# mozilla/mozjpeg

Measured on NVIDIA H100. Metric: megapixels/sec encode (4K RGB q75 4:2:0), higher is better.
Workload: dtype u8 in / int32 DCT / fp32 trellis costs / u8 out

## Files before the change

mozjpeg_b200/csrc/kernels.cu:

```cuda
#include "kernels.cuh"
#include <cuda_fp16.h>
#include <cuda.h>
#include <cstdio>
#include <cstdlib>
#include <type_traits>

namespace b200 {

unsigned long long g_kernel_launches = 0;
#define LAUNCHED() (++g_kernel_launches)

__constant__ uint8_t c_zz[64] = {
   0,  1,  8, 16,  9,  2,  3, 10, 17, 24, 32, 25, 18, 11,  4,  5,
  12, 19, 26, 33, 40, 48, 41, 34, 27, 20, 13,  6,  7, 14, 21, 28,
  35, 42, 49, 56, 57, 50, 43, 36, 29, 22, 15, 23, 30, 37, 44, 51,
  58, 59, 52, 45, 38, 31, 39, 46, 53, 60, 61, 54, 47, 55, 62, 63};
__constant__ uint8_t c_izz[64] = {
   0,  1,  5,  6, 14, 15, 27, 28,  2,  4,  7, 13, 16, 26, 29, 42,
   3,  8, 12, 17, 25, 30, 41, 43,  9, 11, 18, 24, 31, 40, 44, 53,
  10, 19, 23, 32, 39, 45, 52, 54, 20, 22, 33, 38, 46, 51, 55, 60,
  21, 34, 37, 47, 50, 56, 59, 61, 35, 36, 48, 49, 57, 58, 62, 63};
__constant__ unsigned long long c_izz_col[8] = {0x2315140a09030200ull, 0x242216130b080401ull, 0x30252117120c0705ull, 0x312f262018110d06ull, 0x39322e271f19100eull, 0x3a38332d281e1a0full, 0x3e3b37342c291d1bull, 0x3f3d3c36352b2a1cull};
#ifndef FWD_KZ_PACKED
#define FWD_KZ_PACKED 1
#endif
#define ZZ_LIST \
  X(0,0) X(1,1) X(2,8) X(3,16) X(4,9) X(5,2) X(6,3) X(7,10) X(8,17) X(9,24) X(10,32) X(11,25) X(12,18) X(13,11) X(14,4) X(15,5) \
  X(16,12) X(17,19) X(18,26) X(19,33) X(20,40) X(21,48) X(22,41) X(23,34) X(24,27) X(25,20) X(26,13) X(27,6) X(28,7) X(29,14) X(30,21) X(31,28) \
  X(32,35) X(33,42) X(34,49) X(35,56) X(36,57) X(37,50) X(38,43) X(39,36) X(40,29) X(41,22) X(42,15) X(43,23) X(44,30) X(45,37) X(46,44) X(47,51) \
  X(48,58) X(49,59) X(50,52) X(51,45) X(52,38) X(53,31) X(54,39) X(55,46) X(56,53) X(57,60) X(58,61) X(59,54) X(60,47) X(61,55) X(62,62) X(63,63)

#define NAT_LIST Y(1,1) Y(2,5) Y(3,6) Y(4,14) Y(5,15) Y(6,27) Y(7,28) Y(8,2) Y(9,4) Y(10,7) Y(11,13) Y(12,16) Y(13,26) Y(14,29) Y(15,42) Y(16,3) Y(17,8) Y(18,12) Y(19,17) Y(20,25) Y(21,30) Y(22,41) Y(23,43) Y(24,9) Y(25,11) Y(26,18) Y(27,24) Y(28,31) Y(29,40) Y(30,44) Y(31,53) Y(32,10) Y(33,19) Y(34,23) Y(35,32) Y(36,39) Y(37,45) Y(38,52) Y(39,54) Y(40,20) Y(41,22) Y(42,33) Y(43,38) Y(44,46) Y(45,51) Y(46,55) Y(47,60) Y(48,21) Y(49,34) Y(50,37) Y(51,47) Y(52,50) Y(53,56) Y(54,59) Y(55,61) Y(56,35) Y(57,36) Y(58,48) Y(59,49) Y(60,57) Y(61,58) Y(62,62) Y(63,63)

__device__ __forceinline__ int nbits_of(int v) { return 32 - __clz(v); }

template <int SB>
__device__ __forceinline__ int convert_sample(const uint8_t *__restrict__ px, int cs_mode, int comp, int first, int swap)
{
  constexpr int MAXJ = SB == 1 ? 255 : 4095, CENTRE = (MAXJ + 1) / 2;
  auto smp = [&](int k) -> int { return SB == 1 ? (int)px[k] : (int)(reinterpret_cast<const uint16_t *>(px)[k] & 0xFFF); };
  if (cs_mode == 2 || comp == 3) {
    const int k = first + (swap ? 2 - comp : comp);
    return SB == 1 || cs_mode == 2 ? smp(k) : (int)reinterpret_cast<const uint16_t *>(px)[k];
  }
  const int inv = cs_mode == 3 ? MAXJ : 0;
  const int r = smp(first + (swap ? 2 : 0)) ^ inv, g = smp(first + 1) ^ inv, b = smp(first + (swap ? 0 : 2)) ^ inv;
  if (comp == 0) return (19595 * r + 38470 * g + 7471 * b + 32768) >> 16;
  if (comp == 1) return (-11059 * r - 21709 * g + 32768 * b + (CENTRE << 16) + 32767) >> 16;
  return (32768 * r - 27439 * g - 5329 * b + (CENTRE << 16) + 32767) >> 16;
}

#define DESCALE(x, n) (((x) + (1 << ((n) - 1))) >> (n))
template <int PASS, int P1 = 2>
__device__ __forceinline__ void fdct_1d(int &d0, int &d1, int &d2, int &d3, int &d4, int &d5, int &d6, int &d7)
{
  int t0 = d0 + d7, t7 = d0 - d7, t1 = d1 + d6, t6 = d1 - d6;
  int t2 = d2 + d5, t5 = d2 - d5, t3 = d3 + d4, t4 = d3 - d4;
  int t10 = t0 + t3, t13 = t0 - t3, t11 = t1 + t2, t12 = t1 - t2;
  constexpr int SH = PASS == 0 ? 13 - P1 : 13 + P1;
  if (PASS == 0) { d0 = (t10 + t11) << P1; d4 = (t10 - t11) << P1; }
  else { d0 = DESCALE(t10 + t11, P1); d4 = DESCALE(t10 - t11, P1); }
  int z1 = (t12 + t13) * 4433;
  d2 = DESCALE(z1 + t13 * 6270, SH);
  d6 = DESCALE(z1 + t12 * (-15137), SH);
  z1 = t4 + t7; int z2 = t5 + t6, z3 = t4 + t6, z4 = t5 + t7;
  int z5 = (z3 + z4) * 9633;
  t4 *= 2446; t5 *= 16819; t6 *= 25172; t7 *= 12299;
  z1 *= -7373; z2 *= -20995; z3 *= -16069; z4 *= -3196;
  z3 += z5; z4 += z5;
  d7 = DESCALE(t4 + z1 + z3, SH);
  d5 = DESCALE(t5 + z2 + z4, SH);
  d3 = DESCALE(t6 + z2 + z3, SH);
  d1 = DESCALE(t7 + z1 + z4, SH);
}

__device__ __forceinline__ float catmull_rom(int v1, int v2, int v3, int v4, float t, int size)
{
  const int tan1 = (v3 - v1) * size, tan2 = (v4 - v2) * size;
  const float t2 = t * t, t3 = t2 * t;
  const float f1 = 2.f * t3 - 3.f * t2 + 1.f;
  const float f2 = -2.f * t3 + 3.f * t2;
  const float f3 = t3 - 2.f * t2 + t;
  const float f4 = t3 - t2;
  return (float)v2 * f1 + (float)tan1 * f3 + (float)v3 * f2 + (float)tan2 * f4;
}
template <class Acc>
__device__ __forceinline__ void deringing_block(Acc A, int q0, int sum, int cnt)
{
  const int maxsample = 127, size = 64;
  int m = min(min(31, 2 * q0), (maxsample * size - sum) / cnt);
  int maxover = maxsample + m;
  int n = 0;
  do {
    if (A.get(c_zz[n]) < maxsample) { n++; continue; }
    int start = n;
    while (++n < size && A.get(c_zz[n]) >= maxsample) {}
    int end = n;
    int f1 = A.get(c_zz[start >= 1 ? start - 1 : 0]);
    int f2 = A.get(c_zz[start >= 2 ? start - 2 : 0]);
    int l1 = A.get(c_zz[end < size - 1 ? end : size - 1]);
    int l2 = A.get(c_zz[end < size - 2 ? end + 1 : size - 1]);
    int fslope = max(f1 - f2, maxsample - f1);
    int lslope = max(l1 - l2, maxsample - l1);
    if (start == 0) fslope = lslope;
    if (end == size) lslope = fslope;
    int length = end - start;
    float step = 1.f / (float)(length + 1);
    float position = step;
    for (int i = start; i < end; i++, position += step) {
      int tmp = (int)ceilf(catmull_rom(maxsample - fslope, maxsample, maxsample, maxsample - lslope, position, length));
      A.set(c_zz[i], min(tmp, maxover));
    }
    n++;
  } while (n < size);
}
struct LocalAcc { int *d; __device__ int get(int n) const { return d[n]; } __device__ void set(int n, int v) const { d[n] = v; } };
struct PlaneAcc {
  int16_t *p; int pitch;
  __device__ int get(int n) const { return p[(n >> 3) * pitch + (n & 7)]; }
  __device__ void set(int n, int v) const { p[(n >> 3) * pitch + (n & 7)] = (int16_t)v; }
};

__device__ __forceinline__ unsigned quant_one(int x, QuantConst k, int dering)
{
  unsigned a = (unsigned)abs(x) + k.bias;
  int q = (int)(((unsigned long long)a * k.mul) >> k.shift);
  if (dering) q = min(q, 1023);
  return (unsigned)(x < 0 ? -q : q);
}

__device__ __forceinline__ void fdct_ifast_1d(int &d0, int &d1, int &d2, int &d3, int &d4, int &d5, int &d6, int &d7)
{
  int tmp0 = d0 + d7, tmp7 = d0 - d7, tmp1 = d1 + d6, tmp6 = d1 - d6;
  int tmp2 = d2 + d5, tmp5 = d2 - d5, tmp3 = d3 + d4, tmp4 = d3 - d4;
  int tmp10 = tmp0 + tmp3, tmp13 = tmp0 - tmp3, tmp11 = tmp1 + tmp2, tmp12 = tmp1 - tmp2;
  d0 = tmp10 + tmp11; d4 = tmp10 - tmp11;
  int z1 = ((tmp12 + tmp13) * 181) >> 8;
  d2 = tmp13 + z1; d6 = tmp13 - z1;
  tmp10 = tmp4 + tmp5; tmp11 = tmp5 + tmp6; tmp12 = tmp6 + tmp7;
  int z5 = ((tmp10 - tmp12) * 98) >> 8;
  int z2 = ((tmp10 * 139) >> 8) + z5;
  int z4 = ((tmp12 * 334) >> 8) + z5;
  int z3 = (tmp11 * 181) >> 8;
  int z11 = tmp7 + z3, z13 = tmp7 - z3;
  d5 = z13 + z2; d3 = z13 - z2; d1 = z11 + z4; d7 = z11 - z4;
}
__constant__ short c_aanscales[64] = {
  16384, 22725, 21407, 19266, 16384, 12873,  8867,  4520,
  22725, 31521, 29692, 26722, 22725, 17855, 12299,  6270,
  21407, 29692, 27969, 25172, 21407, 16819, 11585,  5906,
  19266, 26722, 25172, 22654, 19266, 15137, 10426,  5315,
  16384, 22725, 21407, 19266, 16384, 12873,  8867,  4520,
  12873, 17855, 16819, 15137, 12873, 10114,  6967,  3552,
   8867, 12299, 11585, 10426,  8867,  6967,  4799,  2446,
   4520,  6270,  5906,  5315,  4520,  3552,  2446,  1247};

__device__ __forceinline__ void fdct_float_1d(float &d0, float &d1, float &d2, float &d3, float &d4, float &d5, float &d6, float &d7)
{
  float tmp0 = d0 + d7, tmp7 = d0 - d7, tmp1 = d1 + d6, tmp6 = d1 - d6;
  float tmp2 = d2 + d5, tmp5 = d2 - d5, tmp3 = d3 + d4, tmp4 = d3 - d4;
  float tmp10 = tmp0 + tmp3, tmp13 = tmp0 - tmp3, tmp11 = tmp1 + tmp2, tmp12 = tmp1 - tmp2;
  d0 = tmp10 + tmp11; d4 = tmp10 - tmp11;
  float z1 = (tmp12 + tmp13) * 0.707106781f;
  d2 = tmp13 + z1; d6 = tmp13 - z1;
  tmp10 = tmp4 + tmp5; tmp11 = tmp5 + tmp6; tmp12 = tmp6 + tmp7;
  float z5 = (tmp10 - tmp12) * 0.382683433f;
  float z2 = 0.541196100f * tmp10 + z5;
  float z4 = 1.306562965f * tmp12 + z5;
  float z3 = tmp11 * 0.707106781f;
  float z11 = tmp7 + z3, z13 = tmp7 - z3;
  d5 = z13 + z2; d3 = z13 - z2; d1 = z11 + z4; d7 = z11 - z4;
}
__device__ __forceinline__ void deringing_block_float(float *data, int q0, float sum, int cnt)
{
  const float maxsample = 127.0f; const int size = 64;
  const int a = min(31, 2 * q0); const float bq = (maxsample * size - sum) / (float)cnt;
  const float maxovershoot = maxsample + ((float)a < bq ? (float)a : bq);
  int n = 0;
  do {
    if (data[c_zz[n]] < maxsample) { n++; continue; }
    int start = n;
    while (++n < size && data[c_zz[n]] >= maxsample) {}
    int end = n;
    float f1 = data[c_zz[start >= 1 ? start - 1 : 0]], f2 = data[c_zz[start >= 2 ? start - 2 : 0]];
    float l1 = data[c_zz[end < size - 1 ? end : size - 1]], l2 = data[c_zz[end < size - 2 ? end + 1 : size - 1]];
    float fslope = fmaxf(f1 - f2, maxsample - f1), lslope = fmaxf(l1 - l2, maxsample - l1);
    if (start == 0) fslope = lslope;
    if (end == size) lslope = fslope;
    int length = end - start;
    float step = 1.f / (float)(length + 1), position = step;
    for (int i = start; i < end; i++, position += step) {
      float tmp = catmull_rom((int)(maxsample - fslope), 127, 127, (int)(maxsample - lslope), position, length);
      data[c_zz[i]] = tmp < maxovershoot ? tmp : maxovershoot;
    }
    n++;
  } while (n < size);
}
__constant__ double c_aan[8] = {1.0, 1.387039845, 1.306562965, 1.175875602, 1.0, 0.785694958, 0.541196100, 0.275899379};

__device__ __forceinline__ unsigned qc_d(const QuantTables *__restrict__ qt, int t, int i) { return qt->q[t][i].d; }
template <int PREC, int DCTM>
__global__ void __launch_bounds__(128) k_forward(Geom g, const uint8_t *__restrict__ src,
                                                 const QuantTables *__restrict__ qt, int dering,
                                                 DcRec *__restrict__ rec, RecLayout rl)
{
  constexpr int CENTRE = 1 << (PREC - 1);
  constexpr int SB = PREC == 8 ? 1 : 2;
  constexpr int P1 = PREC == 8 ? 2 : 1;
  const int ci = blockIdx.z % g.nc, img = blockIdx.z / g.nc;
  const CompGeom &c = g.c[ci];
  int bx = blockIdx.x * blockDim.x + threadIdx.x;
  int by = blockIdx.y;
  if (bx >= c.wib || by >= c.hib) return;
  auto set = [&] { return qset_of(qt, g, img); };
  const uint8_t *base = src + (size_t)img * g.image_stride;
  int ws[64];
  const int comp = g.cs_mode == 1 ? 0 : ci;
  auto component = [&](const uint8_t *px) -> int { return convert_sample<SB>(px, g.cs_mode, comp, g.px_first, g.px_swap); };
#pragma unroll
  for (int y = 0; y < 8; y++) {
    int yo = by * 8 + y;
    int yy = min(yo, c.rows_avail - 1);
    int grp = yy / c.v, sub = yy - grp * c.v;
    int iy0 = grp * g.vmax + sub * c.vx;
#pragma unroll
    for (int x = 0; x < 8; x++) {
      int xo = bx * 8 + x;
      if (g.raw_in) {
        const uint8_t *q = g.plane[ci] + (size_t)img * g.plane_stride[ci] + (size_t)yo * g.plane_pitch[ci] + (size_t)xo * SB;
        ws[8 * y + x] = (SB == 1 ? (int)*q : (int)*reinterpret_cast<const uint16_t *>(q)) - CENTRE;
        continue;
      }
      int sum = 0;
      for (int dv = 0; dv < c.vx; dv++) {
        int iy = min(iy0 + dv, g.H - 1);
        const uint8_t *row = base + (size_t)iy * g.row_pitch;
        for (int du = 0; du < c.hx; du++) {
          int ix = min(xo * c.hx + du, g.W - 1);
          sum += component(row + (size_t)ix * g.in_comps * SB);
        }
      }
      int val;
      if (c.hx == 1 && c.vx == 1) val = sum;
      else if (c.hx == 2 && c.vx == 1) val = (sum + (xo & 1)) >> 1;
      else if (c.hx == 2 && c.vx == 2) val = (sum + 1 + (xo & 1)) >> 2;
      else { int np = c.hx * c.vx; val = (sum + np / 2) / np; }
      ws[8 * y + x] = val - CENTRE;
    }
  }
  int qv[64];
  if (DCTM == 2) {
    float wf[64];
    int sum = 0, cnt = 0;
#pragma unroll
    for (int i = 0; i < 64; i++) { wf[i] = (float)ws[i]; sum += ws[i]; cnt += (ws[i] >= 127); }
    if (dering && cnt != 0 && cnt != 64) deringing_block_float(wf, (int)set()->q[c.qt][0].d >> 3, (float)sum, cnt);
#pragma unroll
    for (int r = 0; r < 8; r++) fdct_float_1d(wf[8 * r], wf[8 * r + 1], wf[8 * r + 2], wf[8 * r + 3], wf[8 * r + 4], wf[8 * r + 5], wf[8 * r + 6], wf[8 * r + 7]);
#pragma unroll
    for (int col = 0; col < 8; col++) fdct_float_1d(wf[col], wf[8 + col], wf[16 + col], wf[24 + col], wf[32 + col], wf[40 + col], wf[48 + col], wf[56 + col]);
    const float *fd = set()->fdiv[c.qt];
#pragma unroll
    for (int i = 0; i < 64; i++) {
      float v = wf[i];
      v = (float)((double)v / c_aan[i & 7]);
      v = (float)((double)v / c_aan[i >> 3]);
      ws[i] = (v >= 0.0f) ? (int)((double)v + 0.5) : (int)((double)v - 0.5);
      int q = (int)(int16_t)(__float2int_rz(wf[i] * fd[i] + 16384.5f) - 16384);
      if (dering) q = max(-1023, min(1023, q));
      qv[i] = q;
    }
  } else {
    if (dering) {
      int sum = 0, cnt = 0;
#pragma unroll
      for (int i = 0; i < 64; i++) { sum += ws[i]; cnt += (ws[i] >= 127); }
      if (cnt != 0 && cnt != 64) {
        int tmp[64];
#pragma unroll
        for (int i = 0; i < 64; i++) tmp[i] = ws[i];
        deringing_block(LocalAcc{tmp}, (int)set()->q[c.qt][0].d >> 3, sum, cnt);
#pragma unroll
        for (int i = 0; i < 64; i++) ws[i] = tmp[i];
      }
    }
    if (DCTM == 1) {
#pragma unroll
      for (int r = 0; r < 8; r++) fdct_ifast_1d(ws[8 * r], ws[8 * r + 1], ws[8 * r + 2], ws[8 * r + 3], ws[8 * r + 4], ws[8 * r + 5], ws[8 * r + 6], ws[8 * r + 7]);
#pragma unroll
      for (int col = 0; col < 8; col++) fdct_ifast_1d(ws[col], ws[8 + col], ws[16 + col], ws[24 + col], ws[32 + col], ws[40 + col], ws[48 + col], ws[56 + col]);
      const IfastConst *ic = set()->ifast[c.qt];
#pragma unroll
      for (int i = 0; i < 64; i++) {
        const int x = ws[i], sc = c_aanscales[i];
        const int a = abs(x);
        int q;
        if (PREC == 8) {
          const IfastConst k = ic[i];
          q = (int)(int16_t)(int)(((unsigned long long)(unsigned)(a + (int)k.corr) * k.recip) >> (k.shift + 32));
        } else {
          const int d = (int)(((long long)((int)qc_d(set(), c.qt, i) >> 3) * sc + (1 << 10)) >> 11);
          q = (int)(int16_t)((a + (d >> 1)) / d);
        }
        if (x < 0) q = (int)(int16_t)(-q);
        if (dering) q = max(-1023, min(1023, q));
        qv[i] = q;
        ws[i] = (int)((x >= 0) ? ((long long)x * 32768 + sc) / (2 * sc) : ((long long)x * 32768 - sc) / (2 * sc));
      }
    } else {
#pragma unroll
      for (int r = 0; r < 8; r++)
        fdct_1d<0, P1>(ws[8 * r], ws[8 * r + 1], ws[8 * r + 2], ws[8 * r + 3], ws[8 * r + 4], ws[8 * r + 5], ws[8 * r + 6], ws[8 * r + 7]);
#pragma unroll
      for (int col = 0; col < 8; col++)
        fdct_1d<1, P1>(ws[col], ws[8 + col], ws[16 + col], ws[24 + col], ws[32 + col], ws[40 + col], ws[48 + col], ws[56 + col]);
    }
  }
  const QuantConst *qc = set()->q[c.qt];
  if (rec) {
    float norm = 0.0f; unsigned long long mask = 0;
#pragma unroll
    for (int i = 1; i < 64; i++) {
      norm += (float)(ws[i] * ws[i]);
      bool nz;
      if (DCTM == 0) nz = quant_one(ws[i], qc[i], dering) != 0u;
      else { const int dq = (int)qc[i].d; nz = abs(ws[i]) >= dq - dq / 2; }
      if (nz) mask |= 1ull << c_izz[i];
    }
    DcRec rr; rr.lambda_dc = norm; rr.raw_dc = (int16_t)ws[0]; rr.nz = (uint8_t)__popcll(mask); rr.pad = 0; rr.nzmask = mask;
    rec[(size_t)img * rl.per_image + rl.comp_off[ci] + (size_t)by * c.wib + bx] = rr;
  }
  size_t blk = ((size_t)img * c.hpad + by) * c.wpad + bx;
  uint4 *dq = reinterpret_cast<uint4 *>(c.coef + blk * 64);
  uint4 *dr = reinterpret_cast<uint4 *>(c.raw + blk * 64);
  unsigned pq[32], pr[32];
#define X(k, n) { unsigned qq = (DCTM == 0 ? quant_one(ws[n], qc[n], dering) : (unsigned)qv[n]) & 0xFFFFu, rr = (unsigned)ws[n] & 0xFFFFu; \
                  if ((k) & 1) { pq[(k) >> 1] |= qq << 16; pr[(k) >> 1] |= rr << 16; } else { pq[(k) >> 1] = qq; pr[(k) >> 1] = rr; } }
  ZZ_LIST
#undef X
#pragma unroll
  for (int v = 0; v < 8; v++) {
    dq[v] = make_uint4(pq[4 * v], pq[4 * v + 1], pq[4 * v + 2], pq[4 * v + 3]);
    dr[v] = make_uint4(pr[4 * v], pr[4 * v + 1], pr[4 * v + 2], pr[4 * v + 3]);
  }
}

template <int PREC> struct WorkT { typedef int16_t type; };
template <> struct WorkT<12> { typedef int type; };
template <> struct WorkT<32> { typedef float type; };
struct Px8 { unsigned w[12]; };
template <int IC, int SB>
__device__ __forceinline__ Px8 load_px8(const uint8_t *__restrict__ base, size_t row_pitch, int iy, int x, int W, bool fast, bool px4 = false, int first = 0)
{
  Px8 r;
  const uint8_t *row = base + (size_t)iy * row_pitch;
  constexpr int NBYTES = 8 * IC * SB;
#pragma unroll
  for (int i = 0; i < 12; i++) r.w[i] = 0;
  if (fast && IC == 3 && px4) {
    unsigned q[16];
    if (SB == 1) {
      const uint4 *p = reinterpret_cast<const uint4 *>(row + (size_t)x * 4);
      const uint4 a = __ldg(p), b = __ldg(p + 1);
      q[0] = a.x; q[1] = a.y; q[2] = a.z; q[3] = a.w; q[4] = b.x; q[5] = b.y; q[6] = b.z; q[7] = b.w;
      if (first) {
#pragma unroll
        for (int i = 0; i < 8; i++) q[i] >>= 8;
      }
#pragma unroll
      for (int g4 = 0; g4 < 2; g4++) {
        const unsigned p0 = q[4 * g4], p1 = q[4 * g4 + 1], p2 = q[4 * g4 + 2], p3 = q[4 * g4 + 3];
        r.w[3 * g4] = __byte_perm(p0, p1, 0x4210);
        r.w[3 * g4 + 1] = __byte_perm(p1, p2, 0x5421);
        r.w[3 * g4 + 2] = __byte_perm(p2, p3, 0x6542);
      }
    } else {
      const uint4 *p = reinterpret_cast<const uint4 *>(row + (size_t)x * 8);
#pragma unroll
      for (int i = 0; i < 4; i++) { const uint4 a = __ldg(p + i); q[4 * i] = a.x; q[4 * i + 1] = a.y; q[4 * i + 2] = a.z; q[4 * i + 3] = a.w; }
#pragma unroll
      for (int k = 0; k < 8; k++) {
        const unsigned lo = q[2 * k], hi = q[2 * k + 1];
        const unsigned c0 = first ? (lo >> 16) : (lo & 0xFFFFu), c1 = first ? (hi & 0xFFFFu) : (lo >> 16), c2 = first ? (hi >> 16) : (hi & 0xFFFFu);
        const unsigned cc[3] = {c0, c1, c2};
#pragma unroll
        for (int c = 0; c < 3; c++) { const int h = 3 * k + c; r.w[h >> 1] |= cc[c] << (16 * (h & 1)); }
      }
    }
    return r;
  }
  if (fast) {
    if (SB == 1) {
      const uint2 *p = reinterpret_cast<const uint2 *>(row + (size_t)x * IC);
#pragma unroll
      for (int i = 0; i < NBYTES / 8; i++) { uint2 a = __ldg(p + i); r.w[2 * i] = a.x; r.w[2 * i + 1] = a.y; }
    } else {
      const uint4 *p = reinterpret_cast<const uint4 *>(row + (size_t)x * IC * 2);
#pragma unroll
      for (int i = 0; i < NBYTES / 16; i++) { uint4 a = __ldg(p + i); r.w[4 * i] = a.x; r.w[4 * i + 1] = a.y; r.w[4 * i + 2] = a.z; r.w[4 * i + 3] = a.w; }
    }
  } else {
    const int pxb = (IC == 3 && px4 ? 4 : IC) * SB, off = (IC == 3 && px4 ? first : 0) * SB;
#pragma unroll
    for (int b = 0; b < NBYTES; b++) {
      int px = b / (IC * SB), rem = b - px * (IC * SB);
      int ix = min(x + px, W - 1);
      r.w[b >> 2] |= (unsigned)row[(size_t)ix * pxb + off + rem] << (8 * (b & 3));
    }
  }
  return r;
}
template <int IC, int SB>
__device__ __forceinline__ int px_sample(const Px8 &r, int px, int ch)
{
  if (SB == 1) { int b = px * IC + ch; return (int)__byte_perm(r.w[b >> 2], 0u, 0x4440 | (b & 3)); }
  int h = px * IC + ch; return (int)((r.w[h >> 1] >> (16 * (h & 1))) & 0xFFFu);
}

__device__ __forceinline__ int quant_fast(int x, uint2 k, int L, int dering)
{
  unsigned a14 = (unsigned)abs(x) * 16384u + k.y;
  int q = (int)(__umulhi(a14, k.x) >> L);
  if (dering) q = min(q, 1023);
  return x < 0 ? -q : q;
}


#ifndef FWD_MASK_SQ
#define FWD_MASK_SQ 1
#endif
#ifndef FWD_MIN_CTAS
#define FWD_MIN_CTAS 6
#endif
template <int HMAX, int VMAX, int NC, bool QFAST, int PREC, int DCTM>
__global__ void __launch_bounds__(128, FWD_MIN_CTAS) k_forward_tile(Geom g, const uint8_t *__restrict__ src,
                                                      const QuantTables *__restrict__ qt, int dering,
                                                      DcRec *__restrict__ rec, RecLayout rl, int write_raw, FwdStats fs,
                                                      const __grid_constant__ CUtensorMap tmap, const int use_tma)
{
  constexpr int TW = 128, TR = 8 * VMAX;
  constexpr int YBW = TW / 8, YB = YBW * VMAX;
  constexpr int CW = TW / HMAX, CBW = CW / 8;
  constexpr int NB = YB + (NC == 3 ? 2 * CBW : 0);
  constexpr int YP = TW + 8, CP = CW + 8;
  constexpr int IC = NC == 3 ? 3 : 1;
  constexpr int SB = PREC == 8 ? 1 : 2;
  constexpr int P1 = PREC == 8 ? 2 : 1;
  constexpr int CENTRE = 1 << (PREC - 1);
  typedef typename WorkT<DCTM == 2 ? 32 : PREC>::type wtype;
  __shared__ __align__(16) int16_t sY[TR * YP];
  __shared__ __align__(16) int16_t sC[NC == 3 ? 2 * 8 * CP : 8];
  __shared__ __align__(16) wtype sW[NB * 72];
  __shared__ __align__(128) unsigned char sIO[NB * 256];
  __shared__ __align__(8) unsigned long long tma_bar;
  __shared__ uint2 sQC[NC][64];
  __shared__ uint2 sMask[NB];
  __shared__ int sQL[NC];
  __shared__ unsigned sHist[NC][HIST_BINS];

  const int tid = threadIdx.x;
  const int tx = blockIdx.x, ty = blockIdx.y, img = blockIdx.z;
  const int x0 = tx * TW, y0 = ty * TR;
  const uint8_t *base = src + (size_t)img * g.image_stride;
  qt = qset_of(qt, g, img);
  if (fs.hist) for (int i = tid; i < NC * HIST_BINS; i += 128) (&sHist[0][0])[i] = 0;

  for (int i = tid; i < NC * 64; i += 128) { int ci = i >> 6, n = i & 63; const QuantConst &k = qt->q[g.c[ci].qt][n]; sQC[ci][n] = make_uint2(k.mul2, k.bias << 14); }
  if (tid < NC) sQL[tid] = qt->L[g.c[tid].qt];

  constexpr int TMA_BOXW = IC == 3 ? 192 : 128, TMA_NBOX = IC == 3 ? 2 : 1;
  static_assert(TMA_NBOX * TMA_BOXW * TR <= NB * 256, "the pixel tile fits the staging buffer it borrows");
  const bool tma_tile = PREC == 8 && use_tma && x0 + TW <= g.W && y0 + TR <= g.H;
  if (tma_tile) {
    const unsigned bar = (unsigned)__cvta_generic_to_shared(&tma_bar);
    if (tid == 0) {
      asm volatile("mbarrier.init.shared::cta.b64 [%0], 1;" :: "r"(bar) : "memory");
      asm volatile("fence.mbarrier_init.release.cluster;" ::: "memory");
      asm volatile("mbarrier.arrive.expect_tx.shared::cta.b64 _, [%0], %1;" :: "r"(bar), "r"((unsigned)(TMA_NBOX * TMA_BOXW * TR)) : "memory");
#pragma unroll
      for (int bx = 0; bx < TMA_NBOX; bx++)
        asm volatile("cp.async.bulk.tensor.3d.shared::cluster.global.mbarrier::complete_tx::bytes [%0], [%1, {%2, %3, %4}], [%5];"
                     :: "r"((unsigned)__cvta_generic_to_shared(sIO + bx * TMA_BOXW * TR)), "l"(reinterpret_cast<unsigned long long>(&tmap)),
                        "r"(x0 * IC + bx * TMA_BOXW), "r"(y0), "r"(g.image_stride ? img : 0), "r"(bar) : "memory");
    }
    __syncthreads();
    {
      unsigned done = 0;
      while (!done)
        asm volatile("{ .reg .pred p; mbarrier.try_wait.parity.shared::cta.b64 p, [%1], 0; selp.u32 %0, 1, 0, p; }" : "=r"(done) : "r"(bar) : "memory");
    }
  }

  {
    const int rg = tid >> 4, seg = tid & 15;
    const int xs = x0 + seg * 8;
    auto tma_px8 = [&](int trow) {
      Px8 r;
#pragma unroll
      for (int i = 0; i < 12; i++) r.w[i] = 0;
      if (IC == 3) {
        const uint2 *q = reinterpret_cast<const uint2 *>(sIO + (seg >> 3) * (TMA_BOXW * TR) + trow * TMA_BOXW + (seg & 7) * 24);
#pragma unroll
        for (int i = 0; i < 3; i++) { const uint2 a = q[i]; r.w[2 * i] = a.x; r.w[2 * i + 1] = a.y; }
      } else {
        const uint2 a = *reinterpret_cast<const uint2 *>(sIO + trow * TMA_BOXW + seg * 8);
        r.w[0] = a.x; r.w[1] = a.y;
      }
      return r;
    };
    if (g.raw_in) {
      auto sample = [&](int cc, int row, int x) -> int {
        const uint8_t *q = g.plane[cc] + (size_t)img * g.plane_stride[cc] + (size_t)row * g.plane_pitch[cc] + (size_t)x * SB;
        return SB == 1 ? (int)*q : (int)*reinterpret_cast<const uint16_t *>(q);
      };
#pragma unroll
      for (int rr = 0; rr < VMAX; rr++) {
        const int row = y0 + rg * VMAX + rr;
        const CompGeom &c0 = g.c[0];
        int16_t yv[8];
#pragma unroll
        for (int px = 0; px < 8; px++) {
          const int x = xs + px;
          yv[px] = (row < c0.hib * 8 && x < c0.wib * 8) ? (int16_t)(sample(0, row, x) - CENTRE) : (int16_t)0;
        }
        *reinterpret_cast<uint4 *>(&sY[(rg * VMAX + rr) * YP + seg * 8]) = *reinterpret_cast<const uint4 *>(yv);
      }
      if (NC == 3) {
        const int row = ty * 8 + rg;
#pragma unroll
        for (int cc = 1; cc <= 2; cc++) {
          const CompGeom &c1 = g.c[cc];
          int16_t cv[8 / HMAX];
#pragma unroll
          for (int i = 0; i < 8 / HMAX; i++) {
            const int x = x0 / HMAX + seg * (8 / HMAX) + i;
            cv[i] = (row < c1.hib * 8 && x < c1.wib * 8) ? (int16_t)(sample(cc, row, x) - CENTRE) : (int16_t)0;
          }
          int16_t *dst = &sC[(cc - 1) * 8 * CP + rg * CP + seg * (8 / HMAX)];
          if (HMAX == 1) *reinterpret_cast<uint4 *>(dst) = *reinterpret_cast<const uint4 *>(cv);
          else *reinterpret_cast<uint2 *>(dst) = *reinterpret_cast<const uint2 *>(cv);
        }
      }
    } else {
    const bool grey_from_rgb = NC == 1 && g.cs_mode == 1;
    const bool px4 = g.in_comps == 4 && (NC == 3 || grey_from_rgb);
    const int pfirst = g.px_first; const bool pswap = g.px_swap != 0;
    const size_t AL = px4 ? 15 : (SB == 1 ? 7 : 15);
    const bool fast = (xs + 8 <= g.W) && ((g.row_pitch & AL) == 0) && ((((size_t)base) & AL) == 0) && !grey_from_rgb;
    if (NC == 1 && grey_from_rgb) {
#pragma unroll
      for (int rr = 0; rr < VMAX; rr++) {
        const int iy = min(y0 + rg * VMAX + rr, g.H - 1);
        const bool f3 = (xs + 8 <= g.W) && ((g.row_pitch & AL) == 0) && ((((size_t)base) & AL) == 0);
        Px8 p = load_px8<3, SB>(base, g.row_pitch, iy, xs, g.W, f3, px4, pfirst);
        int16_t yv[8];
#pragma unroll
        for (int px = 0; px < 8; px++) {
          const int s0 = px_sample<3, SB>(p, px, 0), s2 = px_sample<3, SB>(p, px, 2);
          yv[px] = (int16_t)(((19595 * (pswap ? s2 : s0) + 38470 * px_sample<3, SB>(p, px, 1) + 7471 * (pswap ? s0 : s2) + 32768) >> 16) - CENTRE);
        }
        *reinterpret_cast<uint4 *>(&sY[(rg * VMAX + rr) * YP + seg * 8]) = *reinterpret_cast<const uint4 *>(yv);
      }
    } else {
      auto convert = [&](auto ext_tag) {
      constexpr bool EXT = decltype(ext_tag)::value;
      int sb[8 / HMAX], sr[8 / HMAX];
#pragma unroll
      for (int i = 0; i < 8 / HMAX; i++) { sb[i] = 0; sr[i] = 0; }
      const int last_real = NC == 3 ? g.c[1].rows_avail - 1 - ty * 8 : 8;
      const int er = min(rg, last_real);
#pragma unroll
      for (int rr = 0; rr < VMAX; rr++) {
        const int iy = min(y0 + rg * VMAX + rr, g.H - 1);
        Px8 p = (!EXT && tma_tile) ? tma_px8(rg * VMAX + rr) : load_px8<IC, SB>(base, g.row_pitch, iy, xs, g.W, fast, EXT && px4, EXT ? pfirst : 0);
        int16_t yv[8];
#pragma unroll
        for (int px = 0; px < 8; px++) {
          if (NC == 1) yv[px] = (int16_t)(px_sample<1, SB>(p, px, 0) - CENTRE);
          else {
            const int S0 = px_sample<3, SB>(p, px, 0), G = px_sample<3, SB>(p, px, 1), S2 = px_sample<3, SB>(p, px, 2);
            const int R = (EXT && pswap) ? S2 : S0, B = (EXT && pswap) ? S0 : S2;
            yv[px] = (int16_t)(((19595 * R + 38470 * G + 7471 * B + 32768) >> 16) - CENTRE);
          }
        }
        *reinterpret_cast<uint4 *>(&sY[(rg * VMAX + rr) * YP + seg * 8]) = *reinterpret_cast<const uint4 *>(yv);
        if (NC == 3) {
          if (er != rg) p = (!EXT && tma_tile) ? tma_px8(er * VMAX + rr) : load_px8<IC, SB>(base, g.row_pitch, min(y0 + er * VMAX + rr, g.H - 1), xs, g.W, fast, EXT && px4, EXT ? pfirst : 0);
#pragma unroll
          for (int px = 0; px < 8; px++) {
            const int S0 = px_sample<3, SB>(p, px, 0), G = px_sample<3, SB>(p, px, 1), S2 = px_sample<3, SB>(p, px, 2);
            const int R = (EXT && pswap) ? S2 : S0, B = (EXT && pswap) ? S0 : S2;
            sb[px / HMAX] += (-11059 * R - 21709 * G + 32768 * B + (CENTRE << 16) + 32767) >> 16;
            sr[px / HMAX] += (32768 * R - 27439 * G - 5329 * B + (CENTRE << 16) + 32767) >> 16;
          }
        }
      }
      if (NC == 3) {
        int16_t cbv[8 / HMAX], crv[8 / HMAX];
#pragma unroll
        for (int i = 0; i < 8 / HMAX; i++) {
          const int xo = x0 / HMAX + seg * (8 / HMAX) + i;
          int b = sb[i], r = sr[i];
          if (HMAX == 2 && VMAX == 1) { b = (b + (xo & 1)) >> 1; r = (r + (xo & 1)) >> 1; }
          else if (HMAX == 2 && VMAX == 2) { b = (b + 1 + (xo & 1)) >> 2; r = (r + 1 + (xo & 1)) >> 2; }
          else if (HMAX * VMAX > 1) { b = (b + HMAX * VMAX / 2) / (HMAX * VMAX); r = (r + HMAX * VMAX / 2) / (HMAX * VMAX); }
          cbv[i] = (int16_t)(b - CENTRE); crv[i] = (int16_t)(r - CENTRE);
        }
        int16_t *cb = &sC[rg * CP + seg * (8 / HMAX)], *cr = &sC[8 * CP + rg * CP + seg * (8 / HMAX)];
        if (HMAX == 1) { *reinterpret_cast<uint4 *>(cb) = *reinterpret_cast<const uint4 *>(cbv); *reinterpret_cast<uint4 *>(cr) = *reinterpret_cast<const uint4 *>(crv); }
        else { *reinterpret_cast<uint2 *>(cb) = *reinterpret_cast<const uint2 *>(cbv); *reinterpret_cast<uint2 *>(cr) = *reinterpret_cast<const uint2 *>(crv); }
      }
      };
      if (px4 || pswap) convert(std::true_type{}); else convert(std::false_type{});
    }
    }
  }
  __syncthreads();

  const int j = tid & 7;
#pragma unroll 1
  for (int b = tid >> 3; b < NB; b += 16) {
    int16_t *plane; int pitch, bx, byl;
    if (b < YB) { plane = sY; pitch = YP; byl = b / YBW; bx = b - byl * YBW; }
    else { int cb = b - YB; int which = cb / CBW; plane = sC + which * 8 * CP; pitch = CP; byl = 0; bx = cb - which * CBW; }
    int16_t *rowp = plane + (byl * 8 + j) * pitch + bx * 8;
    const uint4 rv = *reinterpret_cast<const uint4 *>(rowp);
    int d0 = (int)(int16_t)(rv.x & 0xFFFF), d1 = (int)rv.x >> 16, d2 = (int)(int16_t)(rv.y & 0xFFFF), d3 = (int)rv.y >> 16;
    int d4 = (int)(int16_t)(rv.z & 0xFFFF), d5 = (int)rv.z >> 16, d6 = (int)(int16_t)(rv.w & 0xFFFF), d7 = (int)rv.w >> 16;
    if (DCTM == 2) {
      float f0 = (float)d0, f1 = (float)d1, f2 = (float)d2, f3 = (float)d3, f4 = (float)d4, f5 = (float)d5, f6 = (float)d6, f7 = (float)d7;
      float *w = reinterpret_cast<float *>(sW) + b * 72 + j * 8;
      if (dering) {
        int sum = d0 + d1 + d2 + d3 + d4 + d5 + d6 + d7;
        int cnt = (d0 >= 127) + (d1 >= 127) + (d2 >= 127) + (d3 >= 127) + (d4 >= 127) + (d5 >= 127) + (d6 >= 127) + (d7 >= 127);
        sum += __shfl_xor_sync(0xffffffffu, sum, 1); cnt += __shfl_xor_sync(0xffffffffu, cnt, 1);
        sum += __shfl_xor_sync(0xffffffffu, sum, 2); cnt += __shfl_xor_sync(0xffffffffu, cnt, 2);
        sum += __shfl_xor_sync(0xffffffffu, sum, 4); cnt += __shfl_xor_sync(0xffffffffu, cnt, 4);
        if (cnt != 0 && cnt != 64) {
          w[0] = f0; w[1] = f1; w[2] = f2; w[3] = f3; w[4] = f4; w[5] = f5; w[6] = f6; w[7] = f7;
          __syncwarp(0xFFu << (threadIdx.x & 24));
          if (j == 0) {
            const int ci = b < YB ? 0 : (1 + (b - YB) / CBW);
            deringing_block_float(reinterpret_cast<float *>(sW) + b * 72, (int)qt->q[g.c[ci].qt][0].d >> 3, (float)sum, cnt);
          }
          __syncwarp(0xFFu << (threadIdx.x & 24));
          f0 = w[0]; f1 = w[1]; f2 = w[2]; f3 = w[3]; f4 = w[4]; f5 = w[5]; f6 = w[6]; f7 = w[7];
        }
      }
      fdct_float_1d(f0, f1, f2, f3, f4, f5, f6, f7);
      w[0] = f0; w[1] = f1; w[2] = f2; w[3] = f3; w[4] = f4; w[5] = f5; w[6] = f6; w[7] = f7;
      continue;
    }
    if (dering) {
      int sum = d0 + d1 + d2 + d3 + d4 + d5 + d6 + d7;
      int cnt = (d0 >= 127) + (d1 >= 127) + (d2 >= 127) + (d3 >= 127) + (d4 >= 127) + (d5 >= 127) + (d6 >= 127) + (d7 >= 127);
      sum += __shfl_xor_sync(0xffffffffu, sum, 1); cnt += __shfl_xor_sync(0xffffffffu, cnt, 1);
      sum += __shfl_xor_sync(0xffffffffu, sum, 2); cnt += __shfl_xor_sync(0xffffffffu, cnt, 2);
      sum += __shfl_xor_sync(0xffffffffu, sum, 4); cnt += __shfl_xor_sync(0xffffffffu, cnt, 4);
      if (cnt != 0 && cnt != 64) {
        if (j == 0) {
          const int ci = b < YB ? 0 : (1 + (b - YB) / CBW);
          deringing_block(PlaneAcc{plane + (byl * 8) * pitch + bx * 8, pitch}, (int)qt->q[g.c[ci].qt][0].d >> 3, sum, cnt);
        }
        __syncwarp(0xFFu << (threadIdx.x & 24));
        d0 = rowp[0]; d1 = rowp[1]; d2 = rowp[2]; d3 = rowp[3]; d4 = rowp[4]; d5 = rowp[5]; d6 = rowp[6]; d7 = rowp[7];
      }
    }
    if (DCTM == 1) fdct_ifast_1d(d0, d1, d2, d3, d4, d5, d6, d7);
    else fdct_1d<0, P1>(d0, d1, d2, d3, d4, d5, d6, d7);
    if (DCTM == 2) {
    } else if (PREC == 8) {
      uint4 wv;
      wv.x = ((unsigned)d0 & 0xFFFFu) | ((unsigned)d1 << 16); wv.y = ((unsigned)d2 & 0xFFFFu) | ((unsigned)d3 << 16);
      wv.z = ((unsigned)d4 & 0xFFFFu) | ((unsigned)d5 << 16); wv.w = ((unsigned)d6 & 0xFFFFu) | ((unsigned)d7 << 16);
      *reinterpret_cast<uint4 *>(reinterpret_cast<int16_t *>(sW) + b * 72 + j * 8) = wv;
    } else {
      int *w = reinterpret_cast<int *>(sW) + b * 72 + j * 8;
      w[0] = d0; w[1] = d1; w[2] = d2; w[3] = d3; w[4] = d4; w[5] = d5; w[6] = d6; w[7] = d7;
    }
  }
  __syncthreads();

  int16_t *sQ = reinterpret_cast<int16_t *>(sIO);
  int16_t *sR = sQ + NB * 64;
  static_assert(NB % 16 == 0, "whole warps walk the block list in step");
  const int jc = (j + 2 * ((tid >> 3) & 3)) & 7;
  int kz[8];
#pragma unroll
  for (int r = 0; r < 8; r++) {
#if FWD_KZ_PACKED
    kz[r] = (int)((c_izz_col[jc] >> (8 * r)) & 63);
#else
    kz[r] = c_izz[8 * r + jc];
#endif
  }
#pragma unroll 1
  for (int b = tid >> 3; b < NB; b += 16) {
    const wtype *w = sW + b * 72 + jc;
    const int ci = b < YB ? 0 : (1 + (b - YB) / CBW);
    int dd[8], qf[8];
    if (DCTM == 2) {
      float f0 = w[0], f1 = w[8], f2 = w[16], f3 = w[24], f4 = w[32], f5 = w[40], f6 = w[48], f7 = w[56];
      fdct_float_1d(f0, f1, f2, f3, f4, f5, f6, f7);
      const float ff[8] = {f0, f1, f2, f3, f4, f5, f6, f7};
      const float *fd = qt->fdiv[g.c[ci].qt];
#pragma unroll
      for (int r = 0; r < 8; r++) {
        dd[r] = 0;
        if (write_raw) {
          float v = ff[r];
          v = (float)((double)v / c_aan[jc]);
          v = (float)((double)v / c_aan[r]);
          dd[r] = (v >= 0.0f) ? (int)((double)v + 0.5) : (int)((double)v - 0.5);
        }
        const float temp = ff[r] * fd[8 * r + jc];
        int q = (int)(int16_t)(__float2int_rz(temp + 16384.5f) - 16384);
        if (dering) q = max(-1023, min(1023, q));
        qf[r] = q;
      }
    } else if (DCTM == 1) {
      int d0 = w[0], d1 = w[8], d2 = w[16], d3 = w[24], d4 = w[32], d5 = w[40], d6 = w[48], d7 = w[56];
      fdct_ifast_1d(d0, d1, d2, d3, d4, d5, d6, d7);
      const int ws8[8] = {d0, d1, d2, d3, d4, d5, d6, d7};
      const IfastConst *ic = qt->ifast[g.c[ci].qt];
#pragma unroll
      for (int r = 0; r < 8; r++) {
        const int nat = 8 * r + jc;
        dd[r] = 0;
        if (write_raw) { const int x = ws8[r], sc = c_aanscales[nat]; dd[r] = (x >= 0) ? (x * 32768 + sc) / (2 * sc) : (x * 32768 - sc) / (2 * sc); }
        const IfastConst k = ic[nat];
        const int a = abs(ws8[r]);
        int q = (int)(int16_t)(int)(((unsigned long long)(unsigned)(a + (int)k.corr) * k.recip) >> (k.shift + 32));
        if (ws8[r] < 0) q = (int)(int16_t)(-q);
        if (dering) q = max(-1023, min(1023, q));
        qf[r] = q;
      }
    } else {
      int d0 = w[0], d1 = w[8], d2 = w[16], d3 = w[24], d4 = w[32], d5 = w[40], d6 = w[48], d7 = w[56];
      fdct_1d<1, P1>(d0, d1, d2, d3, d4, d5, d6, d7);
      dd[0] = d0; dd[1] = d1; dd[2] = d2; dd[3] = d3; dd[4] = d4; dd[5] = d5; dd[6] = d6; dd[7] = d7;
    }
    const int L = sQL[NC == 1 ? 0 : ci];
    unsigned mlo = 0, mhi = 0;
#pragma unroll
    for (int r = 0; r < 8; r++) {
      const int nat = 8 * r + jc;
      const int k = kz[r];
      int qv;
      if (DCTM != 0) qv = qf[r];
      else if (QFAST) qv = quant_fast(dd[r], sQC[NC == 1 ? 0 : ci][nat], L, dering);
      else qv = (int)(int16_t)quant_one(dd[r], qt->q[g.c[ci].qt][nat], dering);
      sQ[b * 64 + k] = (int16_t)qv;
      sR[b * 64 + k] = (int16_t)dd[r];
      if (!(FWD_MASK_SQ && DCTM == 0)) {
        bool nzv = qv != 0;
        if (DCTM != 0 && rec) { const int dq = (int)qt->q[g.c[ci].qt][nat].d; nzv = abs(dd[r]) >= dq - dq / 2; }
        if (nzv && nat != 0) { if (k < 32) mlo |= 1u << k; else mhi |= 1u << (k - 32); }
      }
    }
    if (PREC == 8 && rec) {
      if (DCTM == 2) __syncwarp();
      int16_t *blk16 = reinterpret_cast<int16_t *>(sW + b * 72);
      int16_t *ww = blk16 + jc;
#pragma unroll
      for (int r = 0; r < 8; r++) ww[8 * r] = (int16_t)dd[r];
      if (FWD_MASK_SQ && DCTM == 0) {
        __syncwarp();
        const uint4 zq = *reinterpret_cast<const uint4 *>(sQ + b * 64 + 8 * j);
        const unsigned zw[4] = {zq.x, zq.y, zq.z, zq.w};
        unsigned m8 = 0;
#pragma unroll
        for (int i = 0; i < 4; i++) {
          const unsigned nz = (((zw[i] & 0x7FFF7FFFu) + 0x7FFF7FFFu) | zw[i]) & 0x80008000u;
          const unsigned t2 = nz >> 15;
          m8 |= ((t2 | (t2 >> 15)) & 3u) << (2 * i);
        }
        if (j == 0) m8 &= ~1u;
        reinterpret_cast<uint8_t *>(&sMask[b])[j] = (uint8_t)m8;
      } else {
      mlo |= __shfl_xor_sync(0xffffffffu, mlo, 1); mhi |= __shfl_xor_sync(0xffffffffu, mhi, 1);
      mlo |= __shfl_xor_sync(0xffffffffu, mlo, 2); mhi |= __shfl_xor_sync(0xffffffffu, mhi, 2);
      mlo |= __shfl_xor_sync(0xffffffffu, mlo, 4); mhi |= __shfl_xor_sync(0xffffffffu, mhi, 4);
      if (j == 0) sMask[b] = make_uint2(mlo, mhi);
      }
    }
  }
  asm volatile("fence.proxy.async.shared::cta;" ::: "memory");
  __syncthreads();

  if (PREC == 8 && rec) {
    for (int b = tid; b < NB; b += 128) {
      int ci, row, col;
      if (b < YB) { ci = 0; int byl = b / YBW; row = ty * VMAX + byl; col = tx * YBW + (b - byl * YBW); }
      else { int cb = b - YB; int which = cb / CBW; ci = 1 + which; row = ty; col = tx * CBW + (cb - which * CBW); }
      const CompGeom &c = g.c[ci];
      if (row >= c.hib || col >= c.wib) continue;
      const int4 *rows = reinterpret_cast<const int4 *>(reinterpret_cast<const int16_t *>(sW + b * 72));
      float norm = 0.0f; int raw_dc = 0;
      const float bias = -8421376.0f;
#pragma unroll
      for (int r = 0; r < 8; r++) {
        const int4 rv = rows[r];
        const unsigned pw[4] = {(unsigned)rv.x, (unsigned)rv.y, (unsigned)rv.z, (unsigned)rv.w};
#pragma unroll
        for (int cp = 0; cp < 4; cp++) {
          const unsigned u = pw[cp] ^ 0x80008000u;
          float2 f = make_float2(__fadd_rn(__uint_as_float(__byte_perm(u, 0x4B000000u, 0x7610)), bias),
                                 __fadd_rn(__uint_as_float(__byte_perm(u, 0x4B000000u, 0x7632)), bias));
          f.x = __fmul_rn(f.x, f.x); f.y = __fmul_rn(f.y, f.y);
          if (r == 0 && cp == 0) raw_dc = (int)(int16_t)(pw[0] & 0xFFFFu); else norm += f.x;
          norm += f.y;
        }
      }
      const uint2 mk = sMask[b];
      DcRec rr; rr.lambda_dc = norm; rr.raw_dc = (int16_t)raw_dc; rr.nz = (uint8_t)(__popc(mk.x) + __popc(mk.y)); rr.pad = 0;
      rr.nzmask = ((unsigned long long)mk.y << 32) | mk.x;
      const size_t ridx = (size_t)img * rl.per_image + rl.comp_off[ci] + (size_t)row * c.wib + col;
      rec[ridx] = rr;
      if (fs.hist) {
        const int16_t *q = sQ + b * 64;
        fs.dcq[ridx] = q[0];
        unsigned long long m;
        if (FWD_MASK_SQ && DCTM == 0) m = rr.nzmask;
        else {
          m = 0;
#pragma unroll
          for (int v = 0; v < 8; v++) {
            const uint4 zq = reinterpret_cast<const uint4 *>(q)[v];
            const unsigned zw[4] = {zq.x, zq.y, zq.z, zq.w};
#pragma unroll
            for (int i = 0; i < 4; i++) {
              const unsigned nz = (((zw[i] & 0x7FFF7FFFu) + 0x7FFF7FFFu) | zw[i]) & 0x80008000u;
              const unsigned t2 = nz >> 15;
              m |= (unsigned long long)((t2 | (t2 >> 15)) & 3u) << (8 * v + 2 * i);
            }
          }
          m &= ~1ull;
        }
        unsigned *h = sHist[NC == 1 ? 0 : ci];
        if (!(m >> 63)) atomicAdd(&h[0], 1u);
        int prev = 0; bool bad = false;
        while (m) {
          const int k = __ffsll((long long)m) - 1;
          m &= m - 1;
          const int run = k - prev - 1; prev = k;
          const int nb = nbits_of(abs((int)q[k]));
          bad |= nb > g.max_coef_bits;
          if (run >> 4) atomicAdd(&h[0xF0], (unsigned)(run >> 4));
          atomicAdd(&h[((run & 15) << 4) + nb], 1u);
        }
        if (bad) atomicOr(&fs.status[img], 2u);
      }
    }
  }

  if (PREC == 8 && fs.hist) {
    __syncthreads();
    for (int i = tid; i < NC * HIST_BINS; i += 128) {
      const unsigned v = (&sHist[0][0])[i];
      const int ci = i / HIST_BINS, sym = i - ci * HIST_BINS;
      if (v) atomicAdd(&fs.hist[(((size_t)img * g.nc + ci) * HIST_SLOTS + 4 + g.c[ci].ac_tbl) * HIST_BINS + sym], v);
    }
  }

  {
    constexpr int NRUN = VMAX + (NC == 3 ? 2 : 0);
    if (tid < NRUN) {
      int ci, row, col0, b0, maxblk;
      if (tid < VMAX) { ci = 0; row = ty * VMAX + tid; col0 = tx * YBW; b0 = tid * YBW; maxblk = YBW; }
      else { const int which = tid - VMAX; ci = 1 + which; row = ty; col0 = tx * CBW; b0 = YB + which * CBW; maxblk = CBW; }
      const CompGeom &c = g.c[ci];
      const int cnt = row < c.hib ? max(0, min(maxblk, c.wib - col0)) : 0;
      if (cnt > 0) {
        const size_t blk = ((size_t)img * c.hpad + row) * c.wpad + col0;
        const unsigned bytes = (unsigned)cnt * 128u;
        if (!fs.hist)
          asm volatile("cp.async.bulk.global.shared::cta.bulk_group [%0], [%1], %2;"
                       :: "l"(c.coef + blk * 64), "r"((unsigned)__cvta_generic_to_shared(sQ + b0 * 64)), "r"(bytes) : "memory");
        if (write_raw)
          asm volatile("cp.async.bulk.global.shared::cta.bulk_group [%0], [%1], %2;"
                       :: "l"(c.raw + blk * 64), "r"((unsigned)__cvta_generic_to_shared(sR + b0 * 64)), "r"(bytes) : "memory");
        asm volatile("cp.async.bulk.commit_group;" ::: "memory");
        asm volatile("cp.async.bulk.wait_group.read 0;" ::: "memory");
      }
    }
  }
}

typedef CUresult (*EncodeTiledFn)(CUtensorMap *, CUtensorMapDataType, cuuint32_t, void *, const cuuint64_t *, const cuuint64_t *, const cuuint32_t *,
                                  const cuuint32_t *, CUtensorMapInterleave, CUtensorMapSwizzle, CUtensorMapL2promotion, CUtensorMapFloatOOBfill);
static EncodeTiledFn tensor_map_encoder()
{
  static EncodeTiledFn fn = [] {
    void *p = nullptr; cudaDriverEntryPointQueryResult q;
    if (cudaGetDriverEntryPoint("cuTensorMapEncodeTiled", &p, cudaEnableDefault, &q) != cudaSuccess || q != cudaDriverEntryPointSuccess) p = nullptr;
    return reinterpret_cast<EncodeTiledFn>(p);
  }();
  return fn;
}
static int make_pixel_tensor_map(const Geom &g, const uint8_t *src, int n, int ic, int tile_rows, CUtensorMap *tm)
{
  static const bool off = getenv("B200JPEG_NO_TMA") != nullptr;
  memset(tm, 0, sizeof *tm);
  EncodeTiledFn enc = tensor_map_encoder();
  if (off || !enc || g.raw_in || !src || g.in_comps != ic || g.px_swap || g.px_first || g.max_coef_bits != 10) return 0;
  if (g.image_stride == 0) n = 1;
  if (((size_t)src & 15) || (g.row_pitch & 15) || (n > 1 && (g.image_stride & 15))) return 0;
  const cuuint64_t dims[3] = {(cuuint64_t)g.W * ic, (cuuint64_t)g.H, (cuuint64_t)n};
  const cuuint64_t strides[2] = {(cuuint64_t)g.row_pitch, (cuuint64_t)(n > 1 ? g.image_stride : ((g.row_pitch * (size_t)g.H + 15) & ~(size_t)15))};
  const cuuint32_t box[3] = {(cuuint32_t)(ic == 3 ? 192 : 128), (cuuint32_t)tile_rows, 1};
  const cuuint32_t estr[3] = {1, 1, 1};
  return enc(tm, CU_TENSOR_MAP_DATA_TYPE_UINT8, 3, const_cast<uint8_t *>(src), dims, strides, box, estr, CU_TENSOR_MAP_INTERLEAVE_NONE,
             CU_TENSOR_MAP_SWIZZLE_NONE, CU_TENSOR_MAP_L2_PROMOTION_L2_128B, CU_TENSOR_MAP_FLOAT_OOB_FILL_NONE) == CUDA_SUCCESS;
}

template <bool QFAST, int PREC, int DCTM>
static void launch_forward_tile(const Geom &g, const uint8_t *src, const QuantTables *qt, int dering, DcRec *rec, const RecLayout &rl, const FwdStats &fs, int n, cudaStream_t s, bool gray, int write_raw)
{
  dim3 grid((g.W + 127) / 128, g.mcu_rows, n);
  CUtensorMap tm;
  const int use_tma = PREC == 8 ? make_pixel_tensor_map(g, src, n, gray ? 1 : 3, 8 * (gray ? 1 : g.vmax), &tm) : (memset(&tm, 0, sizeof tm), 0);
  if (gray) k_forward_tile<1, 1, 1, QFAST, PREC, DCTM><<<grid, 128, 0, s>>>(g, src, qt, dering, rec, rl, write_raw, fs, tm, use_tma);
  else if (g.hmax == 1 && g.vmax == 1) k_forward_tile<1, 1, 3, QFAST, PREC, DCTM><<<grid, 128, 0, s>>>(g, src, qt, dering, rec, rl, write_raw, fs, tm, use_tma);
  else if (g.hmax == 2 && g.vmax == 1) k_forward_tile<2, 1, 3, QFAST, PREC, DCTM><<<grid, 128, 0, s>>>(g, src, qt, dering, rec, rl, write_raw, fs, tm, use_tma);
  else if (g.hmax == 1 && g.vmax == 2) k_forward_tile<1, 2, 3, QFAST, PREC, DCTM><<<grid, 128, 0, s>>>(g, src, qt, dering, rec, rl, write_raw, fs, tm, use_tma);
  else k_forward_tile<2, 2, 3, QFAST, PREC, DCTM><<<grid, 128, 0, s>>>(g, src, qt, dering, rec, rl, write_raw, fs, tm, use_tma);
}
template <int SB>
__global__ void __launch_bounds__(128) k_prep_planes(Geom g, const uint8_t *__restrict__ src, int sf, PlanesOut out)
{
  const int ci = blockIdx.z % g.nc, img = blockIdx.z / g.nc;
  const CompGeom &c = g.c[ci];
  const int xo = blockIdx.x * blockDim.x + threadIdx.x, yo = blockIdx.y;
  if (xo >= c.wib * 8 || yo >= c.hib * 8) return;
  const uint8_t *base = src + (size_t)img * g.image_stride;
  const int comp = g.cs_mode == 1 ? 0 : ci;
  auto at = [&](int y, int x) -> int {
    y = max(0, min(y, g.H - 1)); x = max(0, min(x, g.W - 1));
    return convert_sample<SB>(base + (size_t)y * g.row_pitch + (size_t)x * g.in_comps * SB, g.cs_mode, comp, g.px_first, g.px_swap);
  };
  int val;
  if (c.hx == 1 && c.vx == 1) {
    const int member = at(yo, xo);
    int neigh = -member;
    for (int dy = -1; dy <= 1; dy++) for (int dx = -1; dx <= 1; dx++) neigh += at(yo + dy, xo + dx);
    val = (member * (65536 - sf * 512) + neigh * (sf * 64) + 32768) >> 16;
  } else if (c.hx == 2 && c.vx == 2) {
    const int y = 2 * yo, x = 2 * xo;
    const int member = at(y, x) + at(y, x + 1) + at(y + 1, x) + at(y + 1, x + 1);
    int edge = at(y - 1, x) + at(y - 1, x + 1) + at(y + 2, x) + at(y + 2, x + 1) + at(y, x - 1) + at(y, x + 2) + at(y + 1, x - 1) + at(y + 1, x + 2);
    const int corner = at(y - 1, x - 1) + at(y - 1, x + 2) + at(y + 2, x - 1) + at(y + 2, x + 2);
    val = (member * (16384 - sf * 80) + (2 * edge + corner) * (sf * 16) + 32768) >> 16;
  } else {
    int sum = 0;
    for (int dv = 0; dv < c.vx; dv++) for (int du = 0; du < c.hx; du++) sum += at(yo * c.vx + dv, xo * c.hx + du);
    if (c.hx == 2 && c.vx == 1) val = (sum + (xo & 1)) >> 1;
    else { const int np = c.hx * c.vx; val = (sum + np / 2) / np; }
  }
  uint8_t *dst = out.p[ci] + (size_t)img * out.stride[ci] + (size_t)yo * out.pitch[ci] + (size_t)xo * SB;
  if (SB == 1) *dst = (uint8_t)val; else *reinterpret_cast<uint16_t *>(dst) = (uint16_t)val;
}
void launch_prep_planes(const Geom &g, const uint8_t *src, int smoothing_factor, const PlanesOut &out, int n, cudaStream_t s)
{
  int mw = 0, mh = 0;
  for (int ci = 0; ci < g.nc; ci++) { mw = max(mw, g.c[ci].wib * 8); mh = max(mh, g.c[ci].hib * 8); }
  dim3 grid((mw + 127) / 128, mh, n * g.nc);
  if (g.max_coef_bits == 14) k_prep_planes<2><<<grid, 128, 0, s>>>(g, src, smoothing_factor, out);
  else k_prep_planes<1><<<grid, 128, 0, s>>>(g, src, smoothing_factor, out);
  LAUNCHED();
}

static bool forward_gray(const Geom &g) { return g.nc == 1 && (g.raw_in || g.cs_mode == 1 || (g.cs_mode == 2 && g.in_comps == 1)); }
bool forward_tiled(const Geom &g, int dct_method)
{
  const bool ycc = g.nc == 3 && (g.raw_in || (g.cs_mode == 0 && (g.in_comps == 3 || g.in_comps == 4))) && g.c[0].h == g.hmax && g.c[0].v == g.vmax &&
                   g.c[1].h == 1 && g.c[1].v == 1 && g.c[2].h == 1 && g.c[2].v == 1 && g.hmax <= 2 && g.vmax <= 2;
  static const bool force_generic = getenv("B200JPEG_GENERIC_FORWARD") != nullptr;
  return !force_generic && ((forward_gray(g) && g.hmax == 1 && g.vmax == 1) || ycc) && !(g.max_coef_bits == 14 && dct_method != 0);
}
void launch_forward(const Geom &g, const uint8_t *src, const QuantTables *qt, int qfast, int dct_method, int dering, DcRec *rec, const RecLayout &rl, int keep_raw,
                    const FwdStats &fs, int n, cudaStream_t s)
{
  const int write_raw = rec != nullptr || keep_raw;
  const bool gray = forward_gray(g);
  if (forward_tiled(g, dct_method)) {
    const FwdStats none = {nullptr, nullptr, nullptr};
    if (g.max_coef_bits == 14) {
      if (qfast) launch_forward_tile<true, 12, 0>(g, src, qt, 0, nullptr, rl, none, n, s, gray, 0);
      else launch_forward_tile<false, 12, 0>(g, src, qt, 0, nullptr, rl, none, n, s, gray, 0);
    } else if (dct_method == 2) launch_forward_tile<true, 8, 2>(g, src, qt, dering, rec, rl, fs, n, s, gray, write_raw);
    else if (dct_method == 1) launch_forward_tile<true, 8, 1>(g, src, qt, dering, rec, rl, fs, n, s, gray, write_raw);
    else if (qfast) launch_forward_tile<true, 8, 0>(g, src, qt, dering, rec, rl, fs, n, s, gray, write_raw);
    else launch_forward_tile<false, 8, 0>(g, src, qt, dering, rec, rl, fs, n, s, gray, write_raw);
    LAUNCHED();
    return;
  }
  int mw = 0, mh = 0;
  for (int ci = 0; ci < g.nc; ci++) { mw = max(mw, g.c[ci].wib); mh = max(mh, g.c[ci].hib); }
  dim3 grid((mw + 127) / 128, mh, n * g.nc);
  if (g.max_coef_bits == 14) {
    if (dct_method == 2) k_forward<12, 2><<<grid, 128, 0, s>>>(g, src, qt, 0, nullptr, rl);
    else if (dct_method == 1) k_forward<12, 1><<<grid, 128, 0, s>>>(g, src, qt, 0, nullptr, rl);
    else k_forward<12, 0><<<grid, 128, 0, s>>>(g, src, qt, 0, nullptr, rl);
  }
  else if (dct_method == 2) k_forward<8, 2><<<grid, 128, 0, s>>>(g, src, qt, dering, rec, rl);
  else if (dct_method == 1) k_forward<8, 1><<<grid, 128, 0, s>>>(g, src, qt, dering, rec, rl);
  else k_forward<8, 0><<<grid, 128, 0, s>>>(g, src, qt, dering, rec, rl);
  LAUNCHED();
}

__global__ void __launch_bounds__(256) k_import_coefs(Geom g)
{
  const int ci = blockIdx.y % g.nc, img = blockIdx.y / g.nc;
  const CompGeom &c = g.c[ci];
  const long long nblk = (long long)c.wib * c.hib;
  const long long t = (long long)blockIdx.x * blockDim.x + threadIdx.x;
  if (t >= nblk * 64) return;
  const long long b = t >> 6; const int k = (int)(t & 63);
  const int row = (int)(b / c.wib), col = (int)(b - (long long)row * c.wib);
  const int16_t *src = reinterpret_cast<const int16_t *>(g.plane[ci] + (size_t)img * g.plane_stride[ci] + (size_t)row * g.plane_pitch[ci]) + (size_t)col * 64;
  c.coef[(((size_t)img * c.hpad + row) * c.wpad + col) * 64 + k] = src[c_zz[k]];
}
void launch_import_coefs(const Geom &g, int n, cudaStream_t s)
{
  long long mb = 0;
  for (int ci = 0; ci < g.nc; ci++) mb = max(mb, (long long)g.c[ci].wib * g.c[ci].hib);
  dim3 grid((unsigned)((mb * 64 + 255) / 256), n * g.nc);
  k_import_coefs<<<grid, 256, 0, s>>>(g);
  LAUNCHED();
}

__global__ void k_dummy(Geom g)
{
  const int ci = blockIdx.y % g.nc, img = blockIdx.y / g.nc;
  const CompGeom &c = g.c[ci];
  long long nd_right = (long long)c.hib * (c.wpad - c.wib);
  long long nd = nd_right + (long long)(c.hpad - c.hib) * c.wpad;
  long long t = (long long)blockIdx.x * blockDim.x + threadIdx.x;
  if (t >= nd) return;
  int r, b, srow, scol;
  if (t < nd_right) { r = (int)(t / (c.wpad - c.wib)); b = c.wib + (int)(t % (c.wpad - c.wib)); srow = r; scol = c.wib - 1; }
  else {
    long long u = t - nd_right; r = c.hib + (int)(u / c.wpad); b = (int)(u % c.wpad);
    srow = c.hib - 1; scol = min((b / c.h) * c.h + c.h - 1, c.wib - 1);
  }
  int16_t *dst = c.coef + (((size_t)img * c.hpad + r) * c.wpad + b) * 64;
  int16_t dc = c.coef[(((size_t)img * c.hpad + srow) * c.wpad + scol) * 64];
  uint4 *d4 = reinterpret_cast<uint4 *>(dst);
  d4[0] = make_uint4((unsigned)(uint16_t)dc, 0, 0, 0);
  for (int v = 1; v < 8; v++) d4[v] = make_uint4(0, 0, 0, 0);
}
void launch_dummy(const Geom &g, int n, cudaStream_t s)
{
  long long nd = 0;
  for (int ci = 0; ci < g.nc; ci++) { const CompGeom &c = g.c[ci]; nd = max(nd, (long long)c.hib * (c.wpad - c.wib) + (long long)(c.hpad - c.hib) * c.wpad); }
  if (nd == 0) return;
  dim3 grid((unsigned)((nd + 127) / 128), n * g.nc);
  k_dummy<<<grid, 128, 0, s>>>(g);
  LAUNCHED();
}

struct BlockRef { const int16_t *blk; int sci; int mcu; int k; };

__device__ __forceinline__ const int16_t *block_ptr(const Geom &g, const ScanDesc &sd, int img, long long t, int &sci, long long &mcu, int &k)
{
  mcu = t / sd.bim; k = (int)(t - mcu * sd.bim);
  sci = sd.k_comp[k];
  const CompGeom &c = g.c[sd.ci[sci]];
  long long mrow = mcu / sd.per_row; int mcol = (int)(mcu - mrow * sd.per_row);
  int mh = sd.ncomps == 1 ? 1 : c.v, mw = sd.ncomps == 1 ? 1 : c.h;
  long long row = mrow * mh + sd.k_y[k]; int col = mcol * mw + sd.k_x[k];
  return c.coef + (((size_t)img * c.hpad + row) * c.wpad + col) * 64;
}
__device__ __forceinline__ int prev_dc(const Geom &g, const ScanDesc &sd, int img, long long t, int sci, long long mcu, int k)
{
  long long tp;
  if (k > sd.k_first[sci]) tp = t - 1;
  else if (mcu > 0 && !(sd.ri && mcu % sd.ri == 0)) tp = t - sd.bim + sd.k_count[sci] - 1;
  else return 0;
  int s2, k2; long long m2;
  const int16_t *p = block_ptr(g, sd, img, tp, s2, m2, k2);
  return p[0];
}

template <class Sink, class Load>
__device__ __forceinline__ void walk_seq_chunks(Load ld, int last_dc, Sink &sink)
{
  int r = 0;
#pragma unroll
  for (int v = 0; v < 8; v++) {
    uint4 q = ld(v);
    unsigned w[4] = {q.x, q.y, q.z, q.w};
#pragma unroll
    for (int j = 0; j < 8; j++) {
      int val = (int)(int16_t)((w[j >> 1] >> ((j & 1) * 16)) & 0xFFFF);
      if (v == 0 && j == 0) {
        int temp = val - last_dc, temp2 = temp;
        if (temp < 0) { temp = -temp; temp2--; }
        int nb = nbits_of(temp);
        sink.dc(nb, temp2);
      } else if (val == 0) {
        r++;
      } else {
        while (r > 15) { sink.ac(0xF0, 0, 0); r -= 16; }
        int temp = val, temp2 = val;
        if (temp < 0) { temp = -temp; temp2--; }
        int nb = nbits_of(temp);
        sink.ac((r << 4) + nb, nb, temp2);
        r = 0;
      }
    }
  }
  if (r > 0) sink.ac(0, 0, 0);
}
template <class Sink>
__device__ __forceinline__ void walk_seq_block(const int16_t *__restrict__ blk, int last_dc, Sink &sink)
{
  const uint4 *b4 = reinterpret_cast<const uint4 *>(blk);
  walk_seq_chunks([&](int v) { return b4[v]; }, last_dc, sink);
}

#ifndef SEQ_SPARSE_ENC
#define SEQ_SPARSE_ENC 1
#endif
#ifndef SEQ_SPARSE_STATS
#define SEQ_SPARSE_STATS 0
#endif
__device__ __forceinline__ unsigned long long block_nzmask(const Geom &g, const ScanDesc &sd, const DcRec *__restrict__ rec, const RecLayout &rl,
                                                           int img, int sci, long long mcu, int k)
{
  const int ci = sd.ci[sci];
  const CompGeom &c = g.c[ci];
  const long long mrow = mcu / sd.per_row; const int mcol = (int)(mcu - mrow * sd.per_row);
  const int mh = sd.ncomps == 1 ? 1 : c.v, mw = sd.ncomps == 1 ? 1 : c.h;
  const long long row = mrow * mh + sd.k_y[k]; const int col = mcol * mw + sd.k_x[k];
  return (row < c.hib && col < c.wib) ? rec[(size_t)img * rl.per_image + rl.comp_off[ci] + (size_t)row * c.wib + col].nzmask : 0ull;
}
template <class Sink>
__device__ __forceinline__ void walk_seq_sparse(const int16_t *__restrict__ blk, unsigned long long mask, int last_dc, Sink &sink)
{
  if (mask & 0xFFFF0000ull) asm volatile("prefetch.global.L1 [%0];" :: "l"(blk + 16));
  if (mask & 0xFFFF00000000ull) asm volatile("prefetch.global.L1 [%0];" :: "l"(blk + 32));
  if (mask >> 48) asm volatile("prefetch.global.L1 [%0];" :: "l"(blk + 48));
  {
    int temp = (int)blk[0] - last_dc, temp2 = temp;
    if (temp < 0) { temp = -temp; temp2--; }
    sink.dc(nbits_of(temp), temp2);
  }
  int prev = 0;
  while (mask) {
    const int pos = __ffsll((long long)mask) - 1;
    mask &= mask - 1;
    const int val = blk[pos];
    if (val == 0) continue;
    int r = pos - prev - 1; prev = pos;
    while (r > 15) { sink.ac(0xF0, 0, 0); r -= 16; }
    int temp = val, temp2 = val;
    if (temp < 0) { temp = -temp; temp2--; }
    const int nb = nbits_of(temp);
    sink.ac((r << 4) + nb, nb, temp2);
  }
  if (prev != 63) sink.ac(0, 0, 0);
}


struct ScanPos { int sci, k, mrow, mcol, row, col; unsigned mcu; };
__device__ __forceinline__ void scan_place(const Geom &g, const ScanDesc &sd, ScanPos &p)
{
  const CompGeom &c = g.c[sd.ci[p.sci]];
  const int mh = sd.ncomps == 1 ? 1 : c.v, mw = sd.ncomps == 1 ? 1 : c.h;
  p.row = p.mrow * mh + sd.k_y[p.k]; p.col = p.mcol * mw + sd.k_x[p.k];
}
__device__ __forceinline__ ScanPos scan_coords(const Geom &g, const ScanDesc &sd, long long t)
{
  ScanPos p;
  const unsigned tt = (unsigned)t, bim = (unsigned)sd.bim, per_row = (unsigned)sd.per_row;
  p.mcu = bim == 1 ? tt : tt / bim; p.k = (int)(tt - p.mcu * bim);
  p.sci = sd.k_comp[p.k];
  p.mrow = (int)(p.mcu / per_row); p.mcol = (int)(p.mcu - (unsigned)p.mrow * per_row);
  scan_place(g, sd, p);
  return p;
}
__device__ __forceinline__ int dense_dc(const CompGeom &c, const int16_t *__restrict__ d, int row, int col)
{
  if (row >= c.hib) { row = c.hib - 1; col = min(c.h == 1 ? col : (col / c.h) * c.h + c.h - 1, c.wib - 1); }
  else if (col >= c.wib) col = c.wib - 1;
  return d[(size_t)row * c.wib + col];
}
__device__ __forceinline__ int prev_dc_dense(const Geom &g, const ScanDesc &sd, const int16_t *__restrict__ dimg ,
                                             const RecLayout &rl, const ScanPos &p)
{
  ScanPos q = p;
  if (p.k > sd.k_first[p.sci]) q.k = p.k - 1;
  else if (p.mcu > 0 && !(sd.ri && p.mcu % (unsigned)sd.ri == 0)) {
    q.k = sd.k_first[p.sci] + sd.k_count[p.sci] - 1;
    if (p.mcol > 0) q.mcol = p.mcol - 1; else { q.mrow = p.mrow - 1; q.mcol = sd.per_row - 1; }
  } else return 0;
  scan_place(g, sd, q);
  const int ci = sd.ci[p.sci];
  return dense_dc(g.c[ci], dimg + rl.comp_off[ci], q.row, q.col);
}
template <class Sink>
__device__ __forceinline__ void emit_dc(int dcv, int last_dc, Sink &sink)
{
  int temp = dcv - last_dc, temp2 = temp;
  if (temp < 0) { temp = -temp; temp2--; }
  sink.dc(nbits_of(temp), temp2);
}
template <class Sink>
__device__ __forceinline__ void walk_seq_rec(const Geom &g, const ScanDesc &sd, const uint8_t *__restrict__ sym, const int16_t *__restrict__ dcq, const RecLayout &rl,
                                             int img, long long t, Sink &sink)
{
  const ScanPos sp = scan_coords(g, sd, t);
  const int row = sp.row, col = sp.col;
  const int ci = sd.ci[sp.sci];
  const CompGeom &c = g.c[ci];
  const int16_t *dimg = dcq + (size_t)img * rl.per_image;
  const bool real = row < c.hib && col < c.wib;
  const size_t ridx = (size_t)img * rl.per_image + rl.comp_off[ci] + (real ? (size_t)row * c.wib + col : (size_t)0);
#if SYMREC_SPLIT
  const uint4 *r4 = reinterpret_cast<const uint4 *>(sym + ridx * (SYMREC_BYTES / 2));
  const uint4 *r4hi = reinterpret_cast<const uint4 *>(sym + (size_t)rl.sym_hi + ridx * (SYMREC_BYTES / 2)) - 4;
#else
  const uint4 *r4 = reinterpret_cast<const uint4 *>(sym + ridx * SYMREC_BYTES);
  const uint4 *r4hi = r4;
#endif
  uint4 q0 = make_uint4(1u, 0u, 0u, 0u);
  if (real) q0 = r4[0];
  emit_dc(dense_dc(c, dimg + rl.comp_off[ci], row, col), prev_dc_dense(g, sd, dimg, rl, sp), sink);
// ... 2330 lines not shown
```

Before: 51090.

## Make forward tile kernel persistent with deferred bulk-store waits

Converts the forward DCT/quant tile kernel from one CTA per tile into a persistent grid sized to SM count times occupancy, looping over tiles. Quant constants are reloaded only when the image changes, and histograms are flushed once per image. The TMA mbarrier now tracks a phase parity across tiles. The wait on the bulk coefficient store is moved to the start of the next tile so the store overlaps the next tile's load. The launch-bounds minimum CTAs changes from 6 to 7 for most variants, and optional clock64 phase instrumentation is added behind a macro. Risks include tail imbalance, the extra loop overhead, and register pressure under the tighter bound.

```diff
diff --git a/mozjpeg_b200/csrc/kernels.cu b/mozjpeg_b200/csrc/kernels.cu
--- a/mozjpeg_b200/csrc/kernels.cu
+++ b/mozjpeg_b200/csrc/kernels.cu
@@ -1,6 +1,7 @@
 #include "kernels.cuh"
 #include <cuda_fp16.h>
 #include <cuda.h>
+#include <algorithm>
 #include <cstdio>
 #include <cstdlib>
 #include <type_traits>
@@ -430,13 +431,24 @@
 #define FWD_MASK_SQ 1
 #endif
 #ifndef FWD_MIN_CTAS
-#define FWD_MIN_CTAS 6
+#define FWD_MIN_CTAS 7
+#endif
+#ifndef FWD_PHASE_CLOCKS
+#define FWD_PHASE_CLOCKS 0
+#endif
+enum { FWD_PH_SETUP, FWD_PH_STW, FWD_PH_WAIT, FWD_PH_AB, FWD_PH_C, FWD_PH_D, FWD_PH_D2, FWD_PH_FLUSH, FWD_PH_E, FWD_PH_N };
+#if FWD_PHASE_CLOCKS
+__device__ unsigned long long g_fwd_phase[FWD_PH_N + 1];
+#define FWD_MARK(i) do { if (tid == 0) { const long long t_ = clock64(); ph_acc[i] += t_ - ph_t; ph_t = t_; } } while (0)
+#else
+#define FWD_MARK(i) do { } while (0)
 #endif
 template <int HMAX, int VMAX, int NC, bool QFAST, int PREC, int DCTM>
-__global__ void __launch_bounds__(128, FWD_MIN_CTAS) k_forward_tile(Geom g, const uint8_t *__restrict__ src,
-                                                      const QuantTables *__restrict__ qt, int dering,
+__global__ void __launch_bounds__(128, NC == 3 && HMAX * VMAX == 1 && DCTM == 1 ? 6 : FWD_MIN_CTAS) k_forward_tile(Geom g, const uint8_t *__restrict__ src,
+                                                      const QuantTables *__restrict__ qt_sets, int dering,
                                                       DcRec *__restrict__ rec, RecLayout rl, int write_raw, FwdStats fs,
-                                                      const __grid_constant__ CUtensorMap tmap, const int use_tma)
+                                                      const __grid_constant__ CUtensorMap tmap, const int use_tma,
+                                                      const int ntx, const int tiles_per_img, const int ntiles)
 {
   constexpr int TW = 128, TR = 8 * VMAX;
   constexpr int YBW = TW / 8, YB = YBW * VMAX;
@@ -453,183 +465,221 @@
   __shared__ __align__(16) wtype sW[NB * 72];
   __shared__ __align__(128) unsigned char sIO[NB * 256];
   __shared__ __align__(8) unsigned long long tma_bar;
+  __shared__ unsigned px_parity;
   __shared__ uint2 sQC[NC][64];
   __shared__ uint2 sMask[NB];
   __shared__ int sQL[NC];
   __shared__ unsigned sHist[NC][HIST_BINS];
 
   const int tid = threadIdx.x;
-  const int tx = blockIdx.x, ty = blockIdx.y, img = blockIdx.z;
-  const int x0 = tx * TW, y0 = ty * TR;
-  const uint8_t *base = src + (size_t)img * g.image_stride;
-  qt = qset_of(qt, g, img);
-  if (fs.hist) for (int i = tid; i < NC * HIST_BINS; i += 128) (&sHist[0][0])[i] = 0;
-
-  for (int i = tid; i < NC * 64; i += 128) { int ci = i >> 6, n = i & 63; const QuantConst &k = qt->q[g.c[ci].qt][n]; sQC[ci][n] = make_uint2(k.mul2, k.bias << 14); }
-  if (tid < NC) sQL[tid] = qt->L[g.c[tid].qt];
-
+#if FWD_PHASE_CLOCKS
+  long long ph_t = clock64(), ph_acc[FWD_PH_N] = {};
+#endif
   constexpr int TMA_BOXW = IC == 3 ? 192 : 128, TMA_NBOX = IC == 3 ? 2 : 1;
   static_assert(TMA_NBOX * TMA_BOXW * TR <= NB * 256, "the pixel tile fits the staging buffer it borrows");
-  const bool tma_tile = PREC == 8 && use_tma && x0 + TW <= g.W && y0 + TR <= g.H;
-  if (tma_tile) {
-    const unsigned bar = (unsigned)__cvta_generic_to_shared(&tma_bar);
-    if (tid == 0) {
-      asm volatile("mbarrier.init.shared::cta.b64 [%0], 1;" :: "r"(bar) : "memory");
-      asm volatile("fence.mbarrier_init.release.cluster;" ::: "memory");
-      asm volatile("mbarrier.arrive.expect_tx.shared::cta.b64 _, [%0], %1;" :: "r"(bar), "r"((unsigned)(TMA_NBOX * TMA_BOXW * TR)) : "memory");
-#pragma unroll
-      for (int bx = 0; bx < TMA_NBOX; bx++)
-        asm volatile("cp.async.bulk.tensor.3d.shared::cluster.global.mbarrier::complete_tx::bytes [%0], [%1, {%2, %3, %4}], [%5];"
-                     :: "r"((unsigned)__cvta_generic_to_shared(sIO + bx * TMA_BOXW * TR)), "l"(reinterpret_cast<unsigned long long>(&tmap)),
-                        "r"(x0 * IC + bx * TMA_BOXW), "r"(y0), "r"(g.image_stride ? img : 0), "r"(bar) : "memory");
-    }
+  const unsigned bar = (unsigned)__cvta_generic_to_shared(&tma_bar);
+  if (tid == 0) {
+    asm volatile("mbarrier.init.shared::cta.b64 [%0], 1;" :: "r"(bar) : "memory");
+    asm volatile("fence.mbarrier_init.release.cluster;" ::: "memory");
+    px_parity = 0;
+  }
+  if (fs.hist) for (int i = tid; i < NC * HIST_BINS; i += 128) (&sHist[0][0])[i] = 0;
+  FWD_MARK(FWD_PH_SETUP);
+  constexpr int NRUN = VMAX + (NC == 3 ? 2 : 0);
+
+#pragma unroll 1
+  for (int t = blockIdx.x; t < ntiles; t += gridDim.x) {
+    const int img = t / tiles_per_img, ty = (t - img * tiles_per_img) / ntx, tx = t - img * tiles_per_img - ty * ntx;
+    const int x0 = tx * TW, y0 = ty * TR;
+    const uint8_t *base = src + (size_t)img * g.image_stride;
+    const QuantTables *qt = qset_of(qt_sets, g, img);
+    if (t == (int)blockIdx.x || (t - (int)gridDim.x) / tiles_per_img != img) {
+      for (int i = tid; i < NC * 64; i += 128) { int ci = i >> 6, n = i & 63; const QuantConst &k = qt->q[g.c[ci].qt][n]; sQC[ci][n] = make_uint2(k.mul2, k.bias << 14); }
+      if (tid < NC) sQL[tid] = qt->L[g.c[tid].qt];
+    }
+
+    if (tid < NRUN) asm volatile("cp.async.bulk.wait_group.read 0;" ::: "memory");
     __syncthreads();
-    {
+    FWD_MARK(FWD_PH_STW);
+    const bool tma_tile = PREC == 8 && use_tma && x0 + TW <= g.W && y0 + TR <= g.H;
+    if (tma_tile) {
+      if (tid == 0) {
+        asm volatile("mbarrier.arrive.expect_tx.shared::cta.b64 _, [%0], %1;" :: "r"(bar), "r"((unsigned)(TMA_NBOX * TMA_BOXW * TR)) : "memory");
+#pragma unroll
+        for (int bx = 0; bx < TMA_NBOX; bx++)
+          asm volatile("cp.async.bulk.tensor.3d.shared::cluster.global.mbarrier::complete_tx::bytes [%0], [%1, {%2, %3, %4}], [%5];"
+                       :: "r"((unsigned)__cvta_generic_to_shared(sIO + bx * TMA_BOXW * TR)), "l"(reinterpret_cast<unsigned long long>(&tmap)),
+                          "r"(x0 * IC + bx * TMA_BOXW), "r"(y0), "r"(g.image_stride ? img : 0), "r"(bar) : "memory");
+      }
+      const unsigned parity = px_parity;
       unsigned done = 0;
       while (!done)
-        asm volatile("{ .reg .pred p; mbarrier.try_wait.parity.shared::cta.b64 p, [%1], 0; selp.u32 %0, 1, 0, p; }" : "=r"(done) : "r"(bar) : "memory");
-    }
-  }
-
-  {
-    const int rg = tid >> 4, seg = tid & 15;
-    const int xs = x0 + seg * 8;
-    auto tma_px8 = [&](int trow) {
-      Px8 r;
-#pragma unroll
-      for (int i = 0; i < 12; i++) r.w[i] = 0;
-      if (IC == 3) {
-        const uint2 *q = reinterpret_cast<const uint2 *>(sIO + (seg >> 3) * (TMA_BOXW * TR) + trow * TMA_BOXW + (seg & 7) * 24);
-#pragma unroll
-        for (int i = 0; i < 3; i++) { const uint2 a = q[i]; r.w[2 * i] = a.x; r.w[2 * i + 1] = a.y; }
-      } else {
-        const uint2 a = *reinterpret_cast<const uint2 *>(sIO + trow * TMA_BOXW + seg * 8);
-        r.w[0] = a.x; r.w[1] = a.y;
-      }
-      return r;
-    };
-    if (g.raw_in) {
-      auto sample = [&](int cc, int row, int x) -> int {
-        const uint8_t *q = g.plane[cc] + (size_t)img * g.plane_stride[cc] + (size_t)row * g.plane_pitch[cc] + (size_t)x * SB;
-        return SB == 1 ? (int)*q : (int)*reinterpret_cast<const uint16_t *>(q);
+        asm volatile("{ .reg .pred p; mbarrier.try_wait.parity.shared::cta.b64 p, [%1], %2; selp.u32 %0, 1, 0, p; }" : "=r"(done) : "r"(bar), "r"(parity) : "memory");
+    }
+    FWD_MARK(FWD_PH_WAIT);
+
+    {
+      const int rg = tid >> 4, seg = tid & 15;
+      const int xs = x0 + seg * 8;
+      auto tma_px8 = [&](int trow) {
+        Px8 r;
+#pragma unroll
+        for (int i = 0; i < 12; i++) r.w[i] = 0;
+        if (IC == 3) {
+          const uint2 *q = reinterpret_cast<const uint2 *>(sIO + (seg >> 3) * (TMA_BOXW * TR) + trow * TMA_BOXW + (seg & 7) * 24);
+#pragma unroll
+          for (int i = 0; i < 3; i++) { const uint2 a = q[i]; r.w[2 * i] = a.x; r.w[2 * i + 1] = a.y; }
+        } else {
+          const uint2 a = *reinterpret_cast<const uint2 *>(sIO + trow * TMA_BOXW + seg * 8);
+          r.w[0] = a.x; r.w[1] = a.y;
+        }
+        return r;
       };
-#pragma unroll
-      for (int rr = 0; rr < VMAX; rr++) {
-        const int row = y0 + rg * VMAX + rr;
-        const CompGeom &c0 = g.c[0];
-        int16_t yv[8];
-#pragma unroll
-        for (int px = 0; px < 8; px++) {
-          const int x = xs + px;
-          yv[px] = (row < c0.hib * 8 && x < c0.wib * 8) ? (int16_t)(sample(0, row, x) - CENTRE) : (int16_t)0;
+      if (g.raw_in) {
+        auto sample = [&](int cc, int row, int x) -> int {
+          const uint8_t *q = g.plane[cc] + (size_t)img * g.plane_stride[cc] + (size_t)row * g.plane_pitch[cc] + (size_t)x * SB;
+          return SB == 1 ? (int)*q : (int)*reinterpret_cast<const uint16_t *>(q);
+        };
+#pragma unroll
+        for (int rr = 0; rr < VMAX; rr++) {
+          const int row = y0 + rg * VMAX + rr;
+          const CompGeom &c0 = g.c[0];
+          int16_t yv[8];
+#pragma unroll
+          for (int px = 0; px < 8; px++) {
+            const int x = xs + px;
+            yv[px] = (row < c0.hib * 8 && x < c0.wib * 8) ? (int16_t)(sample(0, row, x) - CENTRE) : (int16_t)0;
+          }
+          *reinterpret_cast<uint4 *>(&sY[(rg * VMAX + rr) * YP + seg * 8]) = *reinterpret_cast<const uint4 *>(yv);
         }
-        *reinterpret_cast<uint4 *>(&sY[(rg * VMAX + rr) * YP + seg * 8]) = *reinterpret_cast<const uint4 *>(yv);
-      }
-      if (NC == 3) {
-        const int row = ty * 8 + rg;
-#pragma unroll
-        for (int cc = 1; cc <= 2; cc++) {
-          const CompGeom &c1 = g.c[cc];
-          int16_t cv[8 / HMAX];
-#pragma unroll
-          for (int i = 0; i < 8 / HMAX; i++) {
-            const int x = x0 / HMAX + seg * (8 / HMAX) + i;
-            cv[i] = (row < c1.hib * 8 && x < c1.wib * 8) ? (int16_t)(sample(cc, row, x) - CENTRE) : (int16_t)0;
-          }
-          int16_t *dst = &sC[(cc - 1) * 8 * CP + rg * CP + seg * (8 / HMAX)];
-          if (HMAX == 1) *reinterpret_cast<uint4 *>(dst) = *reinterpret_cast<const uint4 *>(cv);
-          else *reinterpret_cast<uint2 *>(dst) = *reinterpret_cast<const uint2 *>(cv);
-        }
-      }
-    } else {
-    const bool grey_from_rgb = NC == 1 && g.cs_mode == 1;
-    const bool px4 = g.in_comps == 4 && (NC == 3 || grey_from_rgb);
-    const int pfirst = g.px_first; const bool pswap = g.px_swap != 0;
-    const size_t AL = px4 ? 15 : (SB == 1 ? 7 : 15);
-    const bool fast = (xs + 8 <= g.W) && ((g.row_pitch & AL) == 0) && ((((size_t)base) & AL) == 0) && !grey_from_rgb;
-    if (NC == 1 && grey_from_rgb) {
-#pragma unroll
-      for (int rr = 0; rr < VMAX; rr++) {
-        const int iy = min(y0 + rg * VMAX + rr, g.H - 1);
-        const bool f3 = (xs + 8 <= g.W) && ((g.row_pitch & AL) == 0) && ((((size_t)base) & AL) == 0);
-        Px8 p = load_px8<3, SB>(base, g.row_pitch, iy, xs, g.W, f3, px4, pfirst);
-        int16_t yv[8];
-#pragma unroll
-        for (int px = 0; px < 8; px++) {
-          const int s0 = px_sample<3, SB>(p, px, 0), s2 = px_sample<3, SB>(p, px, 2);
-          yv[px] = (int16_t)(((19595 * (pswap ? s2 : s0) + 38470 * px_sample<3, SB>(p, px, 1) + 7471 * (pswap ? s0 : s2) + 32768) >> 16) - CENTRE);
-        }
-        *reinterpret_cast<uint4 *>(&sY[(rg * VMAX + rr) * YP + seg * 8]) = *reinterpret_cast<const uint4 *>(yv);
-      }
-    } else {
-      auto convert = [&](auto ext_tag) {
-      constexpr bool EXT = decltype(ext_tag)::value;
-      int sb[8 / HMAX], sr[8 / HMAX];
-#pragma unroll
-      for (int i = 0; i < 8 / HMAX; i++) { sb[i] = 0; sr[i] = 0; }
-      const int last_real = NC == 3 ? g.c[1].rows_avail - 1 - ty * 8 : 8;
-      const int er = min(rg, last_real);
-#pragma unroll
-      for (int rr = 0; rr < VMAX; rr++) {
-        const int iy = min(y0 + rg * VMAX + rr, g.H - 1);
-        Px8 p = (!EXT && tma_tile) ? tma_px8(rg * VMAX + rr) : load_px8<IC, SB>(base, g.row_pitch, iy, xs, g.W, fast, EXT && px4, EXT ? pfirst : 0);
-        int16_t yv[8];
-#pragma unroll
-        for (int px = 0; px < 8; px++) {
-          if (NC == 1) yv[px] = (int16_t)(px_sample<1, SB>(p, px, 0) - CENTRE);
-          else {
-            const int S0 = px_sample<3, SB>(p, px, 0), G = px_sample<3, SB>(p, px, 1), S2 = px_sample<3, SB>(p, px, 2);
-            const int R = (EXT && pswap) ? S2 : S0, B = (EXT && pswap) ? S0 : S2;
-            yv[px] = (int16_t)(((19595 * R + 38470 * G + 7471 * B + 32768) >> 16) - CENTRE);
+        if (NC == 3) {
+          const int row = ty * 8 + rg;
+#pragma unroll
+          for (int cc = 1; cc <= 2; cc++) {
+            const CompGeom &c1 = g.c[cc];
+            int16_t cv[8 / HMAX];
+#pragma unroll
+            for (int i = 0; i < 8 / HMAX; i++) {
+              const int x = x0 / HMAX + seg * (8 / HMAX) + i;
+              cv[i] = (row < c1.hib * 8 && x < c1.wib * 8) ? (int16_t)(sample(cc, row, x) - CENTRE) : (int16_t)0;
+            }
+            int16_t *dst = &sC[(cc - 1) * 8 * CP + rg * CP + seg * (8 / HMAX)];
+            if (HMAX == 1) *reinterpret_cast<uint4 *>(dst) = *reinterpret_cast<const uint4 *>(cv);
+            else *reinterpret_cast<uint2 *>(dst) = *reinterpret_cast<const uint2 *>(cv);
           }
         }
-        *reinterpret_cast<uint4 *>(&sY[(rg * VMAX + rr) * YP + seg * 8]) = *reinterpret_cast<const uint4 *>(yv);
-        if (NC == 3) {
-          if (er != rg) p = (!EXT && tma_tile) ? tma_px8(er * VMAX + rr) : load_px8<IC, SB>(base, g.row_pitch, min(y0 + er * VMAX + rr, g.H - 1), xs, g.W, fast, EXT && px4, EXT ? pfirst : 0);
+      } else {
+      const bool grey_from_rgb = NC == 1 && g.cs_mode == 1;
+      const bool px4 = g.in_comps == 4 && (NC == 3 || grey_from_rgb);
+      const int pfirst = g.px_first; const bool pswap = g.px_swap != 0;
+      const size_t AL = px4 ? 15 : (SB == 1 ? 7 : 15);
+      const bool fast = (xs + 8 <= g.W) && ((g.row_pitch & AL) == 0) && ((((size_t)base) & AL) == 0) && !grey_from_rgb;
+      if (NC == 1 && grey_from_rgb) {
+#pragma unroll
+        for (int rr = 0; rr < VMAX; rr++) {
+          const int iy = min(y0 + rg * VMAX + rr, g.H - 1);
+          const bool f3 = (xs + 8 <= g.W) && ((g.row_pitch & AL) == 0) && ((((size_t)base) & AL) == 0);
+          Px8 p = load_px8<3, SB>(base, g.row_pitch, iy, xs, g.W, f3, px4, pfirst);
+          int16_t yv[8];
 #pragma unroll
           for (int px = 0; px < 8; px++) {
-            const int S0 = px_sample<3, SB>(p, px, 0), G = px_sample<3, SB>(p, px, 1), S2 = px_sample<3, SB>(p, px, 2);
-            const int R = (EXT && pswap) ? S2 : S0, B = (EXT && pswap) ? S0 : S2;
-            sb[px / HMAX] += (-11059 * R - 21709 * G + 32768 * B + (CENTRE << 16) + 32767) >> 16;
-            sr[px / HMAX] += (32768 * R - 27439 * G - 5329 * B + (CENTRE << 16) + 32767) >> 16;
+            const int s0 = px_sample<3, SB>(p, px, 0), s2 = px_sample<3, SB>(p, px, 2);
+            yv[px] = (int16_t)(((19595 * (pswap ? s2 : s0) + 38470 * px_sample<3, SB>(p, px, 1) + 7471 * (pswap ? s0 : s2) + 32768) >> 16) - CENTRE);
+          }
+          *reinterpret_cast<uint4 *>(&sY[(rg * VMAX + rr) * YP + seg * 8]) = *reinterpret_cast<const uint4 *>(yv);
+        }
+      } else {
+        auto convert = [&](auto ext_tag) {
+        constexpr bool EXT = decltype(ext_tag)::value;
+        int sb[8 / HMAX], sr[8 / HMAX];
+#pragma unroll
+        for (int i = 0; i < 8 / HMAX; i++) { sb[i] = 0; sr[i] = 0; }
+        const int last_real = NC == 3 ? g.c[1].rows_avail - 1 - ty * 8 : 8;
+        const int er = min(rg, last_real);
+#pragma unroll
+        for (int rr = 0; rr < VMAX; rr++) {
+          const int iy = min(y0 + rg * VMAX + rr, g.H - 1);
+          Px8 p = (!EXT && tma_tile) ? tma_px8(rg * VMAX + rr) : load_px8<IC, SB>(base, g.row_pitch, iy, xs, g.W, fast, EXT && px4, EXT ? pfirst : 0);
+          int16_t yv[8];
+#pragma unroll
+          for (int px = 0; px < 8; px++) {
+            if (NC == 1) yv[px] = (int16_t)(px_sample<1, SB>(p, px, 0) - CENTRE);
+            else {
+              const int S0 = px_sample<3, SB>(p, px, 0), G = px_sample<3, SB>(p, px, 1), S2 = px_sample<3, SB>(p, px, 2);
+              const int R = (EXT && pswap) ? S2 : S0, B = (EXT && pswap) ? S0 : S2;
+              yv[px] = (int16_t)(((19595 * R + 38470 * G + 7471 * B + 32768) >> 16) - CENTRE);
+            }
+          }
+          *reinterpret_cast<uint4 *>(&sY[(rg * VMAX + rr) * YP + seg * 8]) = *reinterpret_cast<const uint4 *>(yv);
+          if (NC == 3) {
+            if (er != rg) p = (!EXT && tma_tile) ? tma_px8(er * VMAX + rr) : load_px8<IC, SB>(base, g.row_pitch, min(y0 + er * VMAX + rr, g.H - 1), xs, g.W, fast, EXT && px4, EXT ? pfirst : 0);
+#pragma unroll
+            for (int px = 0; px < 8; px++) {
+              const int S0 = px_sample<3, SB>(p, px, 0), G = px_sample<3, SB>(p, px, 1), S2 = px_sample<3, SB>(p, px, 2);
+              const int R = (EXT && pswap) ? S2 : S0, B = (EXT && pswap) ? S0 : S2;
+              sb[px / HMAX] += (-11059 * R - 21709 * G + 32768 * B + (CENTRE << 16) + 32767) >> 16;
+              sr[px / HMAX] += (32768 * R - 27439 * G - 5329 * B + (CENTRE << 16) + 32767) >> 16;
+            }
           }
         }
-      }
-      if (NC == 3) {
-        int16_t cbv[8 / HMAX], crv[8 / HMAX];
-#pragma unroll
-        for (int i = 0; i < 8 / HMAX; i++) {
-          const int xo = x0 / HMAX + seg * (8 / HMAX) + i;
-          int b = sb[i], r = sr[i];
-          if (HMAX == 2 && VMAX == 1) { b = (b + (xo & 1)) >> 1; r = (r + (xo & 1)) >> 1; }
-          else if (HMAX == 2 && VMAX == 2) { b = (b + 1 + (xo & 1)) >> 2; r = (r + 1 + (xo & 1)) >> 2; }
-          else if (HMAX * VMAX > 1) { b = (b + HMAX * VMAX / 2) / (HMAX * VMAX); r = (r + HMAX * VMAX / 2) / (HMAX * VMAX); }
-          cbv[i] = (int16_t)(b - CENTRE); crv[i] = (int16_t)(r - CENTRE);
+        if (NC == 3) {
+          int16_t cbv[8 / HMAX], crv[8 / HMAX];
+#pragma unroll
+          for (int i = 0; i < 8 / HMAX; i++) {
+            const int xo = x0 / HMAX + seg * (8 / HMAX) + i;
+            int b = sb[i], r = sr[i];
+            if (HMAX == 2 && VMAX == 1) { b = (b + (xo & 1)) >> 1; r = (r + (xo & 1)) >> 1; }
+            else if (HMAX == 2 && VMAX == 2) { b = (b + 1 + (xo & 1)) >> 2; r = (r + 1 + (xo & 1)) >> 2; }
+            else if (HMAX * VMAX > 1) { b = (b + HMAX * VMAX / 2) / (HMAX * VMAX); r = (r + HMAX * VMAX / 2) / (HMAX * VMAX); }
+            cbv[i] = (int16_t)(b - CENTRE); crv[i] = (int16_t)(r - CENTRE);
+          }
+          int16_t *cb = &sC[rg * CP + seg * (8 / HMAX)], *cr = &sC[8 * CP + rg * CP + seg * (8 / HMAX)];
+          if (HMAX == 1) { *reinterpret_cast<uint4 *>(cb) = *reinterpret_cast<const uint4 *>(cbv); *reinterpret_cast<uint4 *>(cr) = *reinterpret_cast<const uint4 *>(crv); }
+          else { *reinterpret_cast<uint2 *>(cb) = *reinterpret_cast<const uint2 *>(cbv); *reinterpret_cast<uint2 *>(cr) = *reinterpret_cast<const uint2 *>(crv); }
         }
-        int16_t *cb = &sC[rg * CP + seg * (8 / HMAX)], *cr = &sC[8 * CP + rg * CP + seg * (8 / HMAX)];
-        if (HMAX == 1) { *reinterpret_cast<uint4 *>(cb) = *reinterpret_cast<const uint4 *>(cbv); *reinterpret_cast<uint4 *>(cr) = *reinterpret_cast<const uint4 *>(crv); }
-        else { *reinterpret_cast<uint2 *>(cb) = *reinterpret_cast<const uint2 *>(cbv); *reinterpret_cast<uint2 *>(cr) = *reinterpret_cast<const uint2 *>(crv); }
-      }
-      };
-      if (px4 || pswap) convert(std::true_type{}); else convert(std::false_type{});
-    }
-    }
-  }
-  __syncthreads();
-
-  const int j = tid & 7;
+        };
+        if (px4 || pswap) convert(std::true_type{}); else convert(std::false_type{});
+      }
+      }
+    }
+    __syncthreads();
+    FWD_MARK(FWD_PH_AB);
+    if (tid == 0 && tma_tile) px_parity ^= 1;
+
+    const int j = tid & 7;
 #pragma unroll 1
-  for (int b = tid >> 3; b < NB; b += 16) {
-    int16_t *plane; int pitch, bx, byl;
-    if (b < YB) { plane = sY; pitch = YP; byl = b / YBW; bx = b - byl * YBW; }
-    else { int cb = b - YB; int which = cb / CBW; plane = sC + which * 8 * CP; pitch = CP; byl = 0; bx = cb - which * CBW; }
-    int16_t *rowp = plane + (byl * 8 + j) * pitch + bx * 8;
-    const uint4 rv = *reinterpret_cast<const uint4 *>(rowp);
-    int d0 = (int)(int16_t)(rv.x & 0xFFFF), d1 = (int)rv.x >> 16, d2 = (int)(int16_t)(rv.y & 0xFFFF), d3 = (int)rv.y >> 16;
-    int d4 = (int)(int16_t)(rv.z & 0xFFFF), d5 = (int)rv.z >> 16, d6 = (int)(int16_t)(rv.w & 0xFFFF), d7 = (int)rv.w >> 16;
-    if (DCTM == 2) {
-      float f0 = (float)d0, f1 = (float)d1, f2 = (float)d2, f3 = (float)d3, f4 = (float)d4, f5 = (float)d5, f6 = (float)d6, f7 = (float)d7;
-      float *w = reinterpret_cast<float *>(sW) + b * 72 + j * 8;
+    for (int b = tid >> 3; b < NB; b += 16) {
+      int16_t *plane; int pitch, bx, byl;
+      if (b < YB) { plane = sY; pitch = YP; byl = b / YBW; bx = b - byl * YBW; }
+      else { int cb = b - YB; int which = cb / CBW; plane = sC + which * 8 * CP; pitch = CP; byl = 0; bx = cb - which * CBW; }
+      int16_t *rowp = plane + (byl * 8 + j) * pitch + bx * 8;
+      const uint4 rv = *reinterpret_cast<const uint4 *>(rowp);
+      int d0 = (int)(int16_t)(rv.x & 0xFFFF), d1 = (int)rv.x >> 16, d2 = (int)(int16_t)(rv.y & 0xFFFF), d3 = (int)rv.y >> 16;
+      int d4 = (int)(int16_t)(rv.z & 0xFFFF), d5 = (int)rv.z >> 16, d6 = (int)(int16_t)(rv.w & 0xFFFF), d7 = (int)rv.w >> 16;
+      if (DCTM == 2) {
+        float f0 = (float)d0, f1 = (float)d1, f2 = (float)d2, f3 = (float)d3, f4 = (float)d4, f5 = (float)d5, f6 = (float)d6, f7 = (float)d7;
+        float *w = reinterpret_cast<float *>(sW) + b * 72 + j * 8;
+        if (dering) {
+          int sum = d0 + d1 + d2 + d3 + d4 + d5 + d6 + d7;
+          int cnt = (d0 >= 127) + (d1 >= 127) + (d2 >= 127) + (d3 >= 127) + (d4 >= 127) + (d5 >= 127) + (d6 >= 127) + (d7 >= 127);
+          sum += __shfl_xor_sync(0xffffffffu, sum, 1); cnt += __shfl_xor_sync(0xffffffffu, cnt, 1);
+          sum += __shfl_xor_sync(0xffffffffu, sum, 2); cnt += __shfl_xor_sync(0xffffffffu, cnt, 2);
+          sum += __shfl_xor_sync(0xffffffffu, sum, 4); cnt += __shfl_xor_sync(0xffffffffu, cnt, 4);
+          if (cnt != 0 && cnt != 64) {
+            w[0] = f0; w[1] = f1; w[2] = f2; w[3] = f3; w[4] = f4; w[5] = f5; w[6] = f6; w[7] = f7;
+            __syncwarp(0xFFu << (threadIdx.x & 24));
+            if (j == 0) {
+              const int ci = b < YB ? 0 : (1 + (b - YB) / CBW);
+              deringing_block_float(reinterpret_cast<float *>(sW) + b * 72, (int)qt->q[g.c[ci].qt][0].d >> 3, (float)sum, cnt);
+            }
+            __syncwarp(0xFFu << (threadIdx.x & 24));
+            f0 = w[0]; f1 = w[1]; f2 = w[2]; f3 = w[3]; f4 = w[4]; f5 = w[5]; f6 = w[6]; f7 = w[7];
+          }
+        }
+        fdct_float_1d(f0, f1, f2, f3, f4, f5, f6, f7);
+        w[0] = f0; w[1] = f1; w[2] = f2; w[3] = f3; w[4] = f4; w[5] = f5; w[6] = f6; w[7] = f7;
+        continue;
+      }
       if (dering) {
         int sum = d0 + d1 + d2 + d3 + d4 + d5 + d6 + d7;
         int cnt = (d0 >= 127) + (d1 >= 127) + (d2 >= 127) + (d3 >= 127) + (d4 >= 127) + (d5 >= 127) + (d6 >= 127) + (d7 >= 127);
@@ -637,254 +687,246 @@
         sum += __shfl_xor_sync(0xffffffffu, sum, 2); cnt += __shfl_xor_sync(0xffffffffu, cnt, 2);
         sum += __shfl_xor_sync(0xffffffffu, sum, 4); cnt += __shfl_xor_sync(0xffffffffu, cnt, 4);
         if (cnt != 0 && cnt != 64) {
-          w[0] = f0; w[1] = f1; w[2] = f2; w[3] = f3; w[4] = f4; w[5] = f5; w[6] = f6; w[7] = f7;
-          __syncwarp(0xFFu << (threadIdx.x & 24));
           if (j == 0) {
             const int ci = b < YB ? 0 : (1 + (b - YB) / CBW);
-            deringing_block_float(reinterpret_cast<float *>(sW) + b * 72, (int)qt->q[g.c[ci].qt][0].d >> 3, (float)sum, cnt);
+            deringing_block(PlaneAcc{plane + (byl * 8) * pitch + bx * 8, pitch}, (int)qt->q[g.c[ci].qt][0].d >> 3, sum, cnt);
           }
           __syncwarp(0xFFu << (threadIdx.x & 24));
-          f0 = w[0]; f1 = w[1]; f2 = w[2]; f3 = w[3]; f4 = w[4]; f5 = w[5]; f6 = w[6]; f7 = w[7];
+          d0 = rowp[0]; d1 = rowp[1]; d2 = rowp[2]; d3 = rowp[3]; d4 = rowp[4]; d5 = rowp[5]; d6 = rowp[6]; d7 = rowp[7];
         }
       }
-      fdct_float_1d(f0, f1, f2, f3, f4, f5, f6, f7);
-      w[0] = f0; w[1] = f1; w[2] = f2; w[3] = f3; w[4] = f4; w[5] = f5; w[6] = f6; w[7] = f7;
-      continue;
-    }
-    if (dering) {
-      int sum = d0 + d1 + d2 + d3 + d4 + d5 + d6 + d7;
-      int cnt = (d0 >= 127) + (d1 >= 127) + (d2 >= 127) + (d3 >= 127) + (d4 >= 127) + (d5 >= 127) + (d6 >= 127) + (d7 >= 127);
-      sum += __shfl_xor_sync(0xffffffffu, sum, 1); cnt += __shfl_xor_sync(0xffffffffu, cnt, 1);
-      sum += __shfl_xor_sync(0xffffffffu, sum, 2); cnt += __shfl_xor_sync(0xffffffffu, cnt, 2);
-      sum += __shfl_xor_sync(0xffffffffu, sum, 4); cnt += __shfl_xor_sync(0xffffffffu, cnt, 4);
-      if (cnt != 0 && cnt != 64) {
-        if (j == 0) {
-          const int ci = b < YB ? 0 : (1 + (b - YB) / CBW);
-          deringing_block(PlaneAcc{plane + (byl * 8) * pitch + bx * 8, pitch}, (int)qt->q[g.c[ci].qt][0].d >> 3, sum, cnt);
+      if (DCTM == 1) fdct_ifast_1d(d0, d1, d2, d3, d4, d5, d6, d7);
+      else fdct_1d<0, P1>(d0, d1, d2, d3, d4, d5, d6, d7);
+      if (DCTM == 2) {
+      } else if (PREC == 8) {
+        uint4 wv;
+        wv.x = ((unsigned)d0 & 0xFFFFu) | ((unsigned)d1 << 16); wv.y = ((unsigned)d2 & 0xFFFFu) | ((unsigned)d3 << 16);
+        wv.z = ((unsigned)d4 & 0xFFFFu) | ((unsigned)d5 << 16); wv.w = ((unsigned)d6 & 0xFFFFu) | ((unsigned)d7 << 16);
+        *reinterpret_cast<uint4 *>(reinterpret_cast<int16_t *>(sW) + b * 72 + j * 8) = wv;
+      } else {
+        int *w = reinterpret_cast<int *>(sW) + b * 72 + j * 8;
+        w[0] = d0; w[1] = d1; w[2] = d2; w[3] = d3; w[4] = d4; w[5] = d5; w[6] = d6; w[7] = d7;
+      }
+    }
+    __syncthreads();
+    FWD_MARK(FWD_PH_C);
+
+    int16_t *sQ = reinterpret_cast<int16_t *>(sIO);
+    int16_t *sR = sQ + NB * 64;
+    static_assert(NB % 16 == 0, "whole warps walk the block list in step");
+    const int jc = (j + 2 * ((tid >> 3) & 3)) & 7;
+    int kz[8];
+#pragma unroll
+    for (int r = 0; r < 8; r++) {
+#if FWD_KZ_PACKED
+      kz[r] = (int)((c_izz_col[jc] >> (8 * r)) & 63);
+#else
+      kz[r] = c_izz[8 * r + jc];
+#endif
+    }
+#pragma unroll 1
+    for (int b = tid >> 3; b < NB; b += 16) {
+      const wtype *w = sW + b * 72 + jc;
+      const int ci = b < YB ? 0 : (1 + (b - YB) / CBW);
+      int dd[8], qf[8];
+      if (DCTM == 2) {
+        float f0 = w[0], f1 = w[8], f2 = w[16], f3 = w[24], f4 = w[32], f5 = w[40], f6 = w[48], f7 = w[56];
+        fdct_float_1d(f0, f1, f2, f3, f4, f5, f6, f7);
+        const float ff[8] = {f0, f1, f2, f3, f4, f5, f6, f7};
+        const float *fd = qt->fdiv[g.c[ci].qt];
+#pragma unroll
+        for (int r = 0; r < 8; r++) {
+          dd[r] = 0;
+          if (write_raw) {
+            float v = ff[r];
+            v = (float)((double)v / c_aan[jc]);
+            v = (float)((double)v / c_aan[r]);
+            dd[r] = (v >= 0.0f) ? (int)((double)v + 0.5) : (int)((double)v - 0.5);
+          }
+          const float temp = ff[r] * fd[8 * r + jc];
+          int q = (int)(int16_t)(__float2int_rz(temp + 16384.5f) - 16384);
+          if (dering) q = max(-1023, min(1023, q));
+          qf[r] = q;
         }
-        __syncwarp(0xFFu << (threadIdx.x & 24));
-        d0 = rowp[0]; d1 = rowp[1]; d2 = rowp[2]; d3 = rowp[3]; d4 = rowp[4]; d5 = rowp[5]; d6 = rowp[6]; d7 = rowp[7];
-      }
-    }
-    if (DCTM == 1) fdct_ifast_1d(d0, d1, d2, d3, d4, d5, d6, d7);
-    else fdct_1d<0, P1>(d0, d1, d2, d3, d4, d5, d6, d7);
-    if (DCTM == 2) {
-    } else if (PREC == 8) {
-      uint4 wv;
-      wv.x = ((unsigned)d0 & 0xFFFFu) | ((unsigned)d1 << 16); wv.y = ((unsigned)d2 & 0xFFFFu) | ((unsigned)d3 << 16);
-      wv.z = ((unsigned)d4 & 0xFFFFu) | ((unsigned)d5 << 16); wv.w = ((unsigned)d6 & 0xFFFFu) | ((unsigned)d7 << 16);
-      *reinterpret_cast<uint4 *>(reinterpret_cast<int16_t *>(sW) + b * 72 + j * 8) = wv;
-    } else {
-      int *w = reinterpret_cast<int *>(sW) + b * 72 + j * 8;
-      w[0] = d0; w[1] = d1; w[2] = d2; w[3] = d3; w[4] = d4; w[5] = d5; w[6] = d6; w[7] = d7;
-    }
-  }
-  __syncthreads();
-
-  int16_t *sQ = reinterpret_cast<int16_t *>(sIO);
-  int16_t *sR = sQ + NB * 64;
-  static_assert(NB % 16 == 0, "whole warps walk the block list in step");
-  const int jc = (j + 2 * ((tid >> 3) & 3)) & 7;
-  int kz[8];
-#pragma unroll
-  for (int r = 0; r < 8; r++) {
-#if FWD_KZ_PACKED
-    kz[r] = (int)((c_izz_col[jc] >> (8 * r)) & 63);
-#else
-    kz[r] = c_izz[8 * r + jc];
-#endif
-  }
-#pragma unroll 1
-  for (int b = tid >> 3; b < NB; b += 16) {
-    const wtype *w = sW + b * 72 + jc;
-    const int ci = b < YB ? 0 : (1 + (b - YB) / CBW);
-    int dd[8], qf[8];
-    if (DCTM == 2) {
-      float f0 = w[0], f1 = w[8], f2 = w[16], f3 = w[24], f4 = w[32], f5 = w[40], f6 = w[48], f7 = w[56];
-      fdct_float_1d(f0, f1, f2, f3, f4, f5, f6, f7);
-      const float ff[8] = {f0, f1, f2, f3, f4, f5, f6, f7};
-      const float *fd = qt->fdiv[g.c[ci].qt];
-#pragma unroll
-      for (int r = 0; r < 8; r++) {
-        dd[r] = 0;
-        if (write_raw) {
-          float v = ff[r];
-          v = (float)((double)v / c_aan[jc]);
-          v = (float)((double)v / c_aan[r]);
-          dd[r] = (v >= 0.0f) ? (int)((double)v + 0.5) : (int)((double)v - 0.5);
+      } else if (DCTM == 1) {
+        int d0 = w[0], d1 = w[8], d2 = w[16], d3 = w[24], d4 = w[32], d5 = w[40], d6 = w[48], d7 = w[56];
+        fdct_ifast_1d(d0, d1, d2, d3, d4, d5, d6, d7);
+        const int ws8[8] = {d0, d1, d2, d3, d4, d5, d6, d7};
+        const IfastConst *ic = qt->ifast[g.c[ci].qt];
+#pragma unroll
+        for (int r = 0; r < 8; r++) {
+          const int nat = 8 * r + jc;
+          dd[r] = 0;
+          if (write_raw) { const int x = ws8[r], sc = c_aanscales[nat]; dd[r] = (x >= 0) ? (x * 32768 + sc) / (2 * sc) : (x * 32768 - sc) / (2 * sc); }
+          const IfastConst k = ic[nat];
+          const int a = abs(ws8[r]);
+          int q = (int)(int16_t)(int)(((unsigned long long)(unsigned)(a + (int)k.corr) * k.recip) >> (k.shift + 32));
+          if (ws8[r] < 0) q = (int)(int16_t)(-q);
+          if (dering) q = max(-1023, min(1023, q));
+          qf[r] = q;
         }
-        const float temp = ff[r] * fd[8 * r + jc];
-        int q = (int)(int16_t)(__float2int_rz(temp + 16384.5f) - 16384);
-        if (dering) q = max(-1023, min(1023, q));
-        qf[r] = q;
-      }
-    } else if (DCTM == 1) {
-      int d0 = w[0], d1 = w[8], d2 = w[16], d3 = w[24], d4 = w[32], d5 = w[40], d6 = w[48], d7 = w[56];
-      fdct_ifast_1d(d0, d1, d2, d3, d4, d5, d6, d7);
-      const int ws8[8] = {d0, d1, d2, d3, d4, d5, d6, d7};
-      const IfastConst *ic = qt->ifast[g.c[ci].qt];
+      } else {
+        int d0 = w[0], d1 = w[8], d2 = w[16], d3 = w[24], d4 = w[32], d5 = w[40], d6 = w[48], d7 = w[56];
+        fdct_1d<1, P1>(d0, d1, d2, d3, d4, d5, d6, d7);
+        dd[0] = d0; dd[1] = d1; dd[2] = d2; dd[3] = d3; dd[4] = d4; dd[5] = d5; dd[6] = d6; dd[7] = d7;
+      }
+      const int L = sQL[NC == 1 ? 0 : ci];
+      unsigned mlo = 0, mhi = 0;
 #pragma unroll
       for (int r = 0; r < 8; r++) {
         const int nat = 8 * r + jc;
-        dd[r] = 0;
-        if (write_raw) { const int x = ws8[r], sc = c_aanscales[nat]; dd[r] = (x >= 0) ? (x * 32768 + sc) / (2 * sc) : (x * 32768 - sc) / (2 * sc); }
-        const IfastConst k = ic[nat];
-        const int a = abs(ws8[r]);
-        int q = (int)(int16_t)(int)(((unsigned long long)(unsigned)(a + (int)k.corr) * k.recip) >> (k.shift + 32));
-        if (ws8[r] < 0) q = (int)(int16_t)(-q);
-        if (dering) q = max(-1023, min(1023, q));
-        qf[r] = q;
-      }
-    } else {
-      int d0 = w[0], d1 = w[8], d2 = w[16], d3 = w[24], d4 = w[32], d5 = w[40], d6 = w[48], d7 = w[56];
-      fdct_1d<1, P1>(d0, d1, d2, d3, d4, d5, d6, d7);
-      dd[0] = d0; dd[1] = d1; dd[2] = d2; dd[3] = d3; dd[4] = d4; dd[5] = d5; dd[6] = d6; dd[7] = d7;
-    }
-    const int L = sQL[NC == 1 ? 0 : ci];
-    unsigned mlo = 0, mhi = 0;
-#pragma unroll
-    for (int r = 0; r < 8; r++) {
-      const int nat = 8 * r + jc;
-      const int k = kz[r];
-      int qv;
-      if (DCTM != 0) qv = qf[r];
-      else if (QFAST) qv = quant_fast(dd[r], sQC[NC == 1 ? 0 : ci][nat], L, dering);
-      else qv = (int)(int16_t)quant_one(dd[r], qt->q[g.c[ci].qt][nat], dering);
-      sQ[b * 64 + k] = (int16_t)qv;
-      sR[b * 64 + k] = (int16_t)dd[r];
-      if (!(FWD_MASK_SQ && DCTM == 0)) {
-        bool nzv = qv != 0;
-        if (DCTM != 0 && rec) { const int dq = (int)qt->q[g.c[ci].qt][nat].d; nzv = abs(dd[r]) >= dq - dq / 2; }
-        if (nzv && nat != 0) { if (k < 32) mlo |= 1u << k; else mhi |= 1u << (k - 32); }
-      }
-    }
+        const int k = kz[r];
+        int qv;
+        if (DCTM != 0) qv = qf[r];
+        else if (QFAST) qv = quant_fast(dd[r], sQC[NC == 1 ? 0 : ci][nat], L, dering);
+        else qv = (int)(int16_t)quant_one(dd[r], qt->q[g.c[ci].qt][nat], dering);
+        sQ[b * 64 + k] = (int16_t)qv;
+        sR[b * 64 + k] = (int16_t)dd[r];
+        if (!(FWD_MASK_SQ && DCTM == 0)) {
+          bool nzv = qv != 0;
+          if (DCTM != 0 && rec) { const int dq = (int)qt->q[g.c[ci].qt][nat].d; nzv = abs(dd[r]) >= dq - dq / 2; }
+          if (nzv && nat != 0) { if (k < 32) mlo |= 1u << k; else mhi |= 1u << (k - 32); }
+        }
+      }
+      if (PREC == 8 && rec) {
+        if (DCTM == 2) __syncwarp();
+        int16_t *blk16 = reinterpret_cast<int16_t *>(sW + b * 72);
+        int16_t *ww = blk16 + jc;
+#pragma unroll
+        for (int r = 0; r < 8; r++) ww[8 * r] = (int16_t)dd[r];
+        if (FWD_MASK_SQ && DCTM == 0) {
+          __syncwarp();
+          const uint4 zq = *reinterpret_cast<const uint4 *>(sQ + b * 64 + 8 * j);
+          const unsigned zw[4] = {zq.x, zq.y, zq.z, zq.w};
+          unsigned m8 = 0;
+#pragma unroll
+          for (int i = 0; i < 4; i++) {
+            const unsigned nz = (((zw[i] & 0x7FFF7FFFu) + 0x7FFF7FFFu) | zw[i]) & 0x80008000u;
+            const unsigned t2 = nz >> 15;
+            m8 |= ((t2 | (t2 >> 15)) & 3u) << (2 * i);
+          }
+          if (j == 0) m8 &= ~1u;
+          reinterpret_cast<uint8_t *>(&sMask[b])[j] = (uint8_t)m8;
+        } else {
+        mlo |= __shfl_xor_sync(0xffffffffu, mlo, 1); mhi |= __shfl_xor_sync(0xffffffffu, mhi, 1);
+        mlo |= __shfl_xor_sync(0xffffffffu, mlo, 2); mhi |= __shfl_xor_sync(0xffffffffu, mhi, 2);
+        mlo |= __shfl_xor_sync(0xffffffffu, mlo, 4); mhi |= __shfl_xor_sync(0xffffffffu, mhi, 4);
+        if (j == 0) sMask[b] = make_uint2(mlo, mhi);
+        }
+      }
+    }
+    asm volatile("fence.proxy.async.shared::cta;" ::: "memory");
+    __syncthreads();
+    FWD_MARK(FWD_PH_D);
+
     if (PREC == 8 && rec) {
-      if (DCTM == 2) __syncwarp();
-      int16_t *blk16 = reinterpret_cast<int16_t *>(sW + b * 72);
-      int16_t *ww = blk16 + jc;
-#pragma unroll
-      for (int r = 0; r < 8; r++) ww[8 * r] = (int16_t)dd[r];
-      if (FWD_MASK_SQ && DCTM == 0) {
-        __syncwarp();
-        const uint4 zq = *reinterpret_cast<const uint4 *>(sQ + b * 64 + 8 * j);
-        const unsigned zw[4] = {zq.x, zq.y, zq.z, zq.w};
-        unsigned m8 = 0;
-#pragma unroll
-        for (int i = 0; i < 4; i++) {
-          const unsigned nz = (((zw[i] & 0x7FFF7FFFu) + 0x7FFF7FFFu) | zw[i]) & 0x80008000u;
-          const unsigned t2 = nz >> 15;
-          m8 |= ((t2 | (t2 >> 15)) & 3u) << (2 * i);
+      for (int b = tid; b < NB; b += 128) {
+        int ci, row, col;
+        if (b < YB) { ci = 0; int byl = b / YBW; row = ty * VMAX + byl; col = tx * YBW + (b - byl * YBW); }
+        else { int cb = b - YB; int which = cb / CBW; ci = 1 + which; row = ty; col = tx * CBW + (cb - which * CBW); }
+        const CompGeom &c = g.c[ci];
+        if (row >= c.hib || col >= c.wib) continue;
+        const int4 *rows = reinterpret_cast<const int4 *>(reinterpret_cast<const int16_t *>(sW + b * 72));
+        float norm = 0.0f; int raw_dc = 0;
+        const float bias = -8421376.0f;
+#pragma unroll
+        for (int r = 0; r < 8; r++) {
+          const int4 rv = rows[r];
+          const unsigned pw[4] = {(unsigned)rv.x, (unsigned)rv.y, (unsigned)rv.z, (unsigned)rv.w};
+#pragma unroll
+          for (int cp = 0; cp < 4; cp++) {
+            const unsigned u = pw[cp] ^ 0x80008000u;
+            float2 f = make_float2(__fadd_rn(__uint_as_float(__byte_perm(u, 0x4B000000u, 0x7610)), bias),
+                                   __fadd_rn(__uint_as_float(__byte_perm(u, 0x4B000000u, 0x7632)), bias));
+            f.x = __fmul_rn(f.x, f.x); f.y = __fmul_rn(f.y, f.y);
+            if (r == 0 && cp == 0) raw_dc = (int)(int16_t)(pw[0] & 0xFFFFu); else norm += f.x;
+            norm += f.y;
+          }
         }
-        if (j == 0) m8 &= ~1u;
-        reinterpret_cast<uint8_t *>(&sMask[b])[j] = (uint8_t)m8;
-      } else {
-      mlo |= __shfl_xor_sync(0xffffffffu, mlo, 1); mhi |= __shfl_xor_sync(0xffffffffu, mhi, 1);
-      mlo |= __shfl_xor_sync(0xffffffffu, mlo, 2); mhi |= __shfl_xor_sync(0xffffffffu, mhi, 2);
-      mlo |= __shfl_xor_sync(0xffffffffu, mlo, 4); mhi |= __shfl_xor_sync(0xffffffffu, mhi, 4);
-      if (j == 0) sMask[b] = make_uint2(mlo, mhi);
-      }
-    }
-  }
-  asm volatile("fence.proxy.async.shared::cta;" ::: "memory");
-  __syncthreads();
-
-  if (PREC == 8 && rec) {
-    for (int b = tid; b < NB; b += 128) {
-      int ci, row, col;
-      if (b < YB) { ci = 0; int byl = b / YBW; row = ty * VMAX + byl; col = tx * YBW + (b - byl * YBW); }
-      else { int cb = b - YB; int which = cb / CBW; ci = 1 + which; row = ty; col = tx * CBW + (cb - which * CBW); }
-      const CompGeom &c = g.c[ci];
-      if (row >= c.hib || col >= c.wib) continue;
-      const int4 *rows = reinterpret_cast<const int4 *>(reinterpret_cast<const int16_t *>(sW + b * 72));
-      float norm = 0.0f; int raw_dc = 0;
-      const float bias = -8421376.0f;
-#pragma unroll
-      for (int r = 0; r < 8; r++) {
-        const int4 rv = rows[r];
-        const unsigned pw[4] = {(unsigned)rv.x, (unsigned)rv.y, (unsigned)rv.z, (unsigned)rv.w};
-#pragma unroll
-        for (int cp = 0; cp < 4; cp++) {
-          const unsigned u = pw[cp] ^ 0x80008000u;
-          float2 f = make_float2(__fadd_rn(__uint_as_float(__byte_perm(u, 0x4B000000u, 0x7610)), bias),
-                                 __fadd_rn(__uint_as_float(__byte_perm(u, 0x4B000000u, 0x7632)), bias));
-          f.x = __fmul_rn(f.x, f.x); f.y = __fmul_rn(f.y, f.y);
-          if (r == 0 && cp == 0) raw_dc = (int)(int16_t)(pw[0] & 0xFFFFu); else norm += f.x;
-          norm += f.y;
+        const uint2 mk = sMask[b];
+        DcRec rr; rr.lambda_dc = norm; rr.raw_dc = (int16_t)raw_dc; rr.nz = (uint8_t)(__popc(mk.x) + __popc(mk.y)); rr.pad = 0;
+        rr.nzmask = ((unsigned long long)mk.y << 32) | mk.x;
+        const size_t ridx = (size_t)img * rl.per_image + rl.comp_off[ci] + (size_t)row * c.wib + col;
+        rec[ridx] = rr;
+        if (fs.hist) {
+          const int16_t *q = sQ + b * 64;
+          fs.dcq[ridx] = q[0];
+          unsigned long long m;
+          if (FWD_MASK_SQ && DCTM == 0) m = rr.nzmask;
+          else {
+            m = 0;
+#pragma unroll
+            for (int v = 0; v < 8; v++) {
+              const uint4 zq = reinterpret_cast<const uint4 *>(q)[v];
+              const unsigned zw[4] = {zq.x, zq.y, zq.z, zq.w};
+#pragma unroll
+              for (int i = 0; i < 4; i++) {
+                const unsigned nz = (((zw[i] & 0x7FFF7FFFu) + 0x7FFF7FFFu) | zw[i]) & 0x80008000u;
+                const unsigned t2 = nz >> 15;
+                m |= (unsigned long long)((t2 | (t2 >> 15)) & 3u) << (8 * v + 2 * i);
+              }
+            }
+            m &= ~1ull;
+          }
+          unsigned *h = sHist[NC == 1 ? 0 : ci];
+          if (!(m >> 63)) atomicAdd(&h[0], 1u);
+          int prev = 0; bool bad = false;
+          while (m) {
+            const int k = __ffsll((long long)m) - 1;
+            m &= m - 1;
+            const int run = k - prev - 1; prev = k;
+            const int nb = nbits_of(abs((int)q[k]));
+            bad |= nb > g.max_coef_bits;
+            if (run >> 4) atomicAdd(&h[0xF0], (unsigned)(run >> 4));
+            atomicAdd(&h[((run & 15) << 4) + nb], 1u);
+          }
+          if (bad) atomicOr(&fs.status[img], 2u);
         }
       }
-      const uint2 mk = sMask[b];
-      DcRec rr; rr.lambda_dc = norm; rr.raw_dc = (int16_t)raw_dc; rr.nz = (uint8_t)(__popc(mk.x) + __popc(mk.y)); rr.pad = 0;
-      rr.nzmask = ((unsigned long long)mk.y << 32) | mk.x;
-      const size_t ridx = (size_t)img * rl.per_image + rl.comp_off[ci] + (size_t)row * c.wib + col;
-      rec[ridx] = rr;
-      if (fs.hist) {
-        const int16_t *q = sQ + b * 64;
-        fs.dcq[ridx] = q[0];
-        unsigned long long m;
-        if (FWD_MASK_SQ && DCTM == 0) m = rr.nzmask;
-        else {
-          m = 0;
-#pragma unroll
-          for (int v = 0; v < 8; v++) {
-            const uint4 zq = reinterpret_cast<const uint4 *>(q)[v];
-            const unsigned zw[4] = {zq.x, zq.y, zq.z, zq.w};
-#pragma unroll
-            for (int i = 0; i < 4; i++) {
-              const unsigned nz = (((zw[i] & 0x7FFF7FFFu) + 0x7FFF7FFFu) | zw[i]) & 0x80008000u;
-              const unsigned t2 = nz >> 15;
-              m |= (unsigned long long)((t2 | (t2 >> 15)) & 3u) << (8 * v + 2 * i);
-            }
-          }
-          m &= ~1ull;
+    }
+
+    FWD_MARK(FWD_PH_D2);
+
+    if (PREC == 8 && fs.hist && (t + (int)gridDim.x >= ntiles || (t + (int)gridDim.x) / tiles_per_img != img)) {
+      __syncthreads();
+      for (int i = tid; i < NC * HIST_BINS; i += 128) {
+        const unsigned v = (&sHist[0][0])[i];
+        const int ci = i / HIST_BINS, sym = i - ci * HIST_BINS;
+        if (v) { atomicAdd(&fs.hist[(((size_t)img * g.nc + ci) * HIST_SLOTS + 4 + g.c[ci].ac_tbl) * HIST_BINS + sym], v); (&sHist[0][0])[i] = 0; }
+      }
+    }
+    FWD_MARK(FWD_PH_FLUSH);
+
+    {
+      if (tid < NRUN) {
+        int ci, row, col0, b0, maxblk;
+        if (tid < VMAX) { ci = 0; row = ty * VMAX + tid; col0 = tx * YBW; b0 = tid * YBW; maxblk = YBW; }
+        else { const int which = tid - VMAX; ci = 1 + which; row = ty; col0 = tx * CBW; b0 = YB + which * CBW; maxblk = CBW; }
+        const CompGeom &c = g.c[ci];
+        const int cnt = row < c.hib ? max(0, min(maxblk, c.wib - col0)) : 0;
+        if (cnt > 0) {
+          const size_t blk = ((size_t)img * c.hpad + row) * c.wpad + col0;
+          const unsigned bytes = (unsigned)cnt * 128u;
+          if (!fs.hist)
+            asm volatile("cp.async.bulk.global.shared::cta.bulk_group [%0], [%1], %2;"
+                         :: "l"(c.coef + blk * 64), "r"((unsigned)__cvta_generic_to_shared(sQ + b0 * 64)), "r"(bytes) : "memory");
+          if (write_raw)
+            asm volatile("cp.async.bulk.global.shared::cta.bulk_group [%0], [%1], %2;"
+                         :: "l"(c.raw + blk * 64), "r"((unsigned)__cvta_generic_to_shared(sR + b0 * 64)), "r"(bytes) : "memory");
+          asm volatile("cp.async.bulk.commit_group;" ::: "memory");
         }
-        unsigned *h = sHist[NC == 1 ? 0 : ci];
-        if (!(m >> 63)) atomicAdd(&h[0], 1u);
-        int prev = 0; bool bad = false;
-        while (m) {
-          const int k = __ffsll((long long)m) - 1;
-          m &= m - 1;
-          const int run = k - prev - 1; prev = k;
-          const int nb = nbits_of(abs((int)q[k]));
-          bad |= nb > g.max_coef_bits;
-          if (run >> 4) atomicAdd(&h[0xF0], (unsigned)(run >> 4));
-          atomicAdd(&h[((run & 15) << 4) + nb], 1u);
-        }
-        if (bad) atomicOr(&fs.status[img], 2u);
-      }
-    }
-  }
-
-  if (PREC == 8 && fs.hist) {
-    __syncthreads();
-    for (int i = tid; i < NC * HIST_BINS; i += 128) {
-      const unsigned v = (&sHist[0][0])[i];
-      const int ci = i / HIST_BINS, sym = i - ci * HIST_BINS;
-      if (v) atomicAdd(&fs.hist[(((size_t)img * g.nc + ci) * HIST_SLOTS + 4 + g.c[ci].ac_tbl) * HIST_BINS + sym], v);
-    }
-  }
-
-  {
-    constexpr int NRUN = VMAX + (NC == 3 ? 2 : 0);
-    if (tid < NRUN) {
-      int ci, row, col0, b0, maxblk;
-      if (tid < VMAX) { ci = 0; row = ty * VMAX + tid; col0 = tx * YBW; b0 = tid * YBW; maxblk = YBW; }
-      else { const int which = tid - VMAX; ci = 1 + which; row = ty; col0 = tx * CBW; b0 = YB + which * CBW; maxblk = CBW; }
-      const CompGeom &c = g.c[ci];
-      const int cnt = row < c.hib ? max(0, min(maxblk, c.wib - col0)) : 0;
-      if (cnt > 0) {
-        const size_t blk = ((size_t)img * c.hpad + row) * c.wpad + col0;
-        const unsigned bytes = (unsigned)cnt * 128u;
-        if (!fs.hist)
-          asm volatile("cp.async.bulk.global.shared::cta.bulk_group [%0], [%1], %2;"
-                       :: "l"(c.coef + blk * 64), "r"((unsigned)__cvta_generic_to_shared(sQ + b0 * 64)), "r"(bytes) : "memory");
-        if (write_raw)
-          asm volatile("cp.async.bulk.global.shared::cta.bulk_group [%0], [%1], %2;"
-                       :: "l"(c.raw + blk * 64), "r"((unsigned)__cvta_generic_to_shared(sR + b0 * 64)), "r"(bytes) : "memory");
-        asm volatile("cp.async.bulk.commit_group;" ::: "memory");
-        asm volatile("cp.async.bulk.wait_group.read 0;" ::: "memory");
-      }
-    }
-  }
+      }
+    }
+    FWD_MARK(FWD_PH_E);
+  }
+  if (tid < NRUN) asm volatile("cp.async.bulk.wait_group.read 0;" ::: "memory");
+#if FWD_PHASE_CLOCKS
+  if (tid == 0) {
+#pragma unroll
+    for (int i = 0; i < FWD_PH_N; i++) atomicAdd(&g_fwd_phase[i], (unsigned long long)ph_acc[i]);
+    atomicAdd(&g_fwd_phase[FWD_PH_N], (unsigned long long)((ntiles - (int)blockIdx.x + (int)gridDim.x - 1) / (int)gridDim.x));
+  }
+#endif
 }
 
 typedef CUresult (*EncodeTiledFn)(CUtensorMap *, CUtensorMapDataType, cuuint32_t, void *, const cuuint64_t *, const cuuint64_t *, const cuuint32_t *,
@@ -914,17 +956,48 @@
              CU_TENSOR_MAP_SWIZZLE_NONE, CU_TENSOR_MAP_L2_PROMOTION_L2_128B, CU_TENSOR_MAP_FLOAT_OOB_FILL_NONE) == CUDA_SUCCESS;
 }
 
+#if FWD_PHASE_CLOCKS
+static void print_phase_clocks()
+{
+  unsigned long long h[FWD_PH_N + 1];
+  if (cudaMemcpyFromSymbol(h, g_fwd_phase, sizeof h) != cudaSuccess || h[FWD_PH_N] == 0) return;
+  static const char *const names[FWD_PH_N] = {"setup", "store_wait", "tma_wait", "ab", "c", "d", "d2", "flush", "e"};
+  fprintf(stderr, "{\"fwd_phase_cycles_per_tile\": {");
+  for (int i = 0; i < FWD_PH_N; i++) fprintf(stderr, "%s\"%s\": %.1f", i ? ", " : "", names[i], (double)h[i] / (double)h[FWD_PH_N]);
+  fprintf(stderr, "}, \"tiles\": %llu}\n", h[FWD_PH_N]);
+}
+#endif
+
+template <int HMAX, int VMAX, int NC, bool QFAST, int PREC, int DCTM>
+static void launch_tiles(const Geom &g, const uint8_t *src, const QuantTables *qt, int dering, DcRec *rec, const RecLayout &rl, int write_raw,
+                         const FwdStats &fs, const CUtensorMap &tm, int use_tma, int n, cudaStream_t s)
+{
+  static const int per_sm = [] {
+    int b = 0;
+    cudaOccupancyMaxActiveBlocksPerMultiprocessor(&b, k_forward_tile<HMAX, VMAX, NC, QFAST, PREC, DCTM>, 128, 0);
+    return b > 0 ? b : 1;
+  }();
+  int dev = 0, sms = 0;
+  cudaGetDevice(&dev);
+  cudaDeviceGetAttribute(&sms, cudaDevAttrMultiProcessorCount, dev);
+  const int ntx = (g.W + 127) / 128, tiles = ntx * g.mcu_rows * n;
+  const int grid = std::min(tiles, std::max(sms, 1) * per_sm);
+  k_forward_tile<HMAX, VMAX, NC, QFAST, PREC, DCTM><<<grid, 128, 0, s>>>(g, src, qt, dering, rec, rl, write_raw, fs, tm, use_tma, ntx, ntx * g.mcu_rows, tiles);
+}
+
 template <bool QFAST, int PREC, int DCTM>
 static void launch_forward_tile(const Geom &g, const uint8_t *src, const QuantTables *qt, int dering, DcRec *rec, const RecLayout &rl, const FwdStats &fs, int n, cudaStream_t s, bool gray, int write_raw)
 {
-  dim3 grid((g.W + 127) / 128, g.mcu_rows, n);
+#if FWD_PHASE_CLOCKS
+  print_phase_clocks();
+#endif
   CUtensorMap tm;
   const int use_tma = PREC == 8 ? make_pixel_tensor_map(g, src, n, gray ? 1 : 3, 8 * (gray ? 1 : g.vmax), &tm) : (memset(&tm, 0, sizeof tm), 0);
-  if (gray) k_forward_tile<1, 1, 1, QFAST, PREC, DCTM><<<grid, 128, 0, s>>>(g, src, qt, dering, rec, rl, write_raw, fs, tm, use_tma);
-  else if (g.hmax == 1 && g.vmax == 1) k_forward_tile<1, 1, 3, QFAST, PREC, DCTM><<<grid, 128, 0, s>>>(g, src, qt, dering, rec, rl, write_raw, fs, tm, use_tma);
-  else if (g.hmax == 2 && g.vmax == 1) k_forward_tile<2, 1, 3, QFAST, PREC, DCTM><<<grid, 128, 0, s>>>(g, src, qt, dering, rec, rl, write_raw, fs, tm, use_tma);
-  else if (g.hmax == 1 && g.vmax == 2) k_forward_tile<1, 2, 3, QFAST, PREC, DCTM><<<grid, 128, 0, s>>>(g, src, qt, dering, rec, rl, write_raw, fs, tm, use_tma);
-  else k_forward_tile<2, 2, 3, QFAST, PREC, DCTM><<<grid, 128, 0, s>>>(g, src, qt, dering, rec, rl, write_raw, fs, tm, use_tma);
+  if (gray) launch_tiles<1, 1, 1, QFAST, PREC, DCTM>(g, src, qt, dering, rec, rl, write_raw, fs, tm, use_tma, n, s);
+  else if (g.hmax == 1 && g.vmax == 1) launch_tiles<1, 1, 3, QFAST, PREC, DCTM>(g, src, qt, dering, rec, rl, write_raw, fs, tm, use_tma, n, s);
+  else if (g.hmax == 2 && g.vmax == 1) launch_tiles<2, 1, 3, QFAST, PREC, DCTM>(g, src, qt, dering, rec, rl, write_raw, fs, tm, use_tma, n, s);
+  else if (g.hmax == 1 && g.vmax == 2) launch_tiles<1, 2, 3, QFAST, PREC, DCTM>(g, src, qt, dering, rec, rl, write_raw, fs, tm, use_tma, n, s);
+  else launch_tiles<2, 2, 3, QFAST, PREC, DCTM>(g, src, qt, dering, rec, rl, write_raw, fs, tm, use_tma, n, s);
 }
 template <int SB>
 __global__ void __launch_bounds__(128) k_prep_planes(Geom g, const uint8_t *__restrict__ src, int sf, PlanesOut out)
```

New measurement: 52350, median of 6. 2.5% higher.
